# sIncerass/MVLPT

Measured on AMD Instinct MI355X. Metric: prompt-tuning images/sec (fwd+bwd), ViT-B/16 bs=256, 1/2/4/8 MI355X, higher is better.
Workload: dtype fp16; 1 GPU; BASELINE configs[1]: MVLPT coop head, ViT-B/16, 100 classes (caltech101 token table), n_ctx=16 n_vpt=0, text L=77, class token middle; text_positions_evaluated=77, step_pipelining=True, grad_precision=split_grad, layernorm_folding=both towers, residual_stream=packed fp16 + byte (image tower without prompts / backward), cu_partition=none (towers share every compute unit), per_gpu_batch=256, global_batch=256, parallelism=dp1, text_tower=replicated per GPU

## Files before the change

include/mvlpt_hip.h:

```cpp
#ifndef MVLPT_HIP_H
#define MVLPT_HIP_H
#include <stdint.h>
#ifdef __cplusplus
extern "C" {
#endif

typedef void* mvlpt_stream_t;

enum { MVLPT_DT_F32 = 0, MVLPT_DT_F16 = 1, MVLPT_DT_BF16 = 2 };
enum { MVLPT_LABEL_INT64 = 0, MVLPT_LABEL_PROB_F32 = 1 };
enum { MVLPT_ERR_ARG = -1, MVLPT_ERR_HIP = -2, MVLPT_ERR_STATE = -3, MVLPT_ERR_UNSUPPORTED = -4 };

typedef struct MvlptArch {
  int image_resolution, patch_size, vision_width, vision_layers, vision_heads;
  int context_length, text_width, text_layers, text_heads;
  int embed_dim;
  int compute_dtype;
} MvlptArch;

enum { MVLPT_PREC_FAST = 0, MVLPT_PREC_SPLIT_GRAD = 1, MVLPT_PREC_SPLIT_ALL = 2 };

int mvlpt_create(const MvlptArch* arch, void** handle);
int mvlpt_set_precision(void* handle, int mode);
int mvlpt_set_ln_fold(void* handle, int mode, int min_rows);
int mvlpt_set_resid_packed(void* handle, int on);
int mvlpt_set_vpt_dropout(void* handle, const float* masks, int n_layers, int batch, int n_vpt, int width);
int mvlpt_trim(void* handle);
int mvlpt_debug_checksums(void* handle, int enable, unsigned long long* host_out, int max_out);
int mvlpt_destroy(void* handle);
const char* mvlpt_last_error(void* handle);
const char* mvlpt_version(void);

int mvlpt_stream_create_cus(int cu_first, int cu_count, mvlpt_stream_t* stream);
int mvlpt_stream_destroy(mvlpt_stream_t stream);
int mvlpt_stream_cus(mvlpt_stream_t stream);

int mvlpt_load_frozen(void* handle, const char* name, const void* dev_ptr, int dtype, const int64_t* shape, int ndim,
                      mvlpt_stream_t stream);
int mvlpt_frozen_ready(void* handle);

int mvlpt_image_fwd(void* handle, const void* image, int image_dtype, const float* vpt, const float* vpt_deep, int n_vpt,
                    int n_deep, int B, float* feat_out, int save_for_bwd, mvlpt_stream_t stream);
int mvlpt_image_bwd(void* handle, const float* dfeat, float* dvpt, float* dvpt_deep, mvlpt_stream_t stream);

int mvlpt_text_fwd(void* handle, const float* prefix, const float* suffix, const float* ctx, int ctx_per_class, int n_ctx,
                   const int32_t* layout, const int32_t* eot, int C, int L, float* feat_out, int save_for_bwd,
                   mvlpt_stream_t stream);
int mvlpt_text_fwd_grouped(void* handle, const float* prefix, const float* suffix, const float* ctx, int n_ctx, const int32_t* layout,
                           const int32_t* eot, int G, int C, int L, float* feat_out, int save_for_bwd, mvlpt_stream_t stream);
int mvlpt_text_fwd_ranged(void* handle, const float* prefix, const float* suffix, const float* ctx, int n_ctx, const int32_t* layout,
                          const int32_t* eot, const int32_t* class_lo, const int32_t* class_hi, int G, int C, int L, float* feat_out,
                          int save_for_bwd, mvlpt_stream_t stream);
int mvlpt_text_bwd(void* handle, const float* dfeat, float* dctx, mvlpt_stream_t stream);
int mvlpt_text_workspace_bytes(void* handle, int C_total, int L, int save_for_bwd, int64_t* out);

enum { MVLPT_TEXT_MIN_L = 3 };
int mvlpt_text_encode_tokens(void* handle, const int32_t* ids, int ld, int S, int L, float* feat_out, mvlpt_stream_t stream);
int mvlpt_text_ensemble(const float* feats, int T, int C, int e, float* out, mvlpt_stream_t stream);

int mvlpt_logits_fwd(void* handle, const float* img_feat, const float* txt_feat, float logit_scale_exp, const int32_t* task_lo,
                     const int32_t* task_hi, int B, int C, float* logits, mvlpt_stream_t stream);
int mvlpt_logits_bwd(void* handle, const float* dlogits, float* dimg, float* dtxt, mvlpt_stream_t stream);
int mvlpt_logits_grouped_fwd(void* handle, const float* img, const float* txt, float logit_scale_exp, int G, int C, float* logits,
                             mvlpt_stream_t stream);
int mvlpt_logits_grouped_bwd(void* handle, const float* dlogits, float* dtxt, mvlpt_stream_t stream);
int mvlpt_logits_ranged_fwd(void* handle, const float* img, const float* txt, float logit_scale_exp, const int32_t* class_lo,
                            const int32_t* class_hi, int G, int C, float* logits, mvlpt_stream_t stream);
int mvlpt_logits_ranged_bwd(void* handle, const float* dlogits, float* dtxt, float* dimg, mvlpt_stream_t stream);

int mvlpt_cross_entropy(void* handle, const float* logits, const void* labels, int label_kind, int B, int C, float* loss,
                        float* dlogits, float* ncorrect, mvlpt_stream_t stream);

int mvlpt_op_gemm(int dtype, int epi, const void* A, const void* Bt, int M, int N, int K, const float* bias, const void* aux,
                  const float* resid, void* out, void* out2, mvlpt_stream_t stream);
int mvlpt_op_gemm_ex(int dtype, int epi, const void* A, const void* Bt, int M, int N, int K, const float* bias, const void* aux,
                     const float* resid, void* out, void* out2, int a_split, int lda, int ldo, int ldb, int w8_exp, int out_lo8,
                     mvlpt_stream_t stream);
enum { MVLPT_GEMM_BT_128x128_R2 = 1, MVLPT_GEMM_BT_128x128_R4 = 2, MVLPT_GEMM_BT_256x128_R3 = 3, MVLPT_GEMM_BT_256x256_R2 = 4,
       MVLPT_GEMM_PHASED = 5, MVLPT_GEMM_PC = 6, MVLPT_GEMM_PCP = 7 };
int mvlpt_op_gemm_route(int dtype, int epi, int a_split, int M, int N, int K, int fold_ntp, mvlpt_stream_t stream, int* tile_m,
                        int* tile_n, int* ring);
int mvlpt_op_gemm_split(int dtype, int epi, const void* A, const void* Bt, int M, int N, int K, const float* bias, const void* aux,
                        const float* resid, void* out, void* out2, mvlpt_stream_t stream);
int mvlpt_op_layernorm_fwd_split(int out_dtype, const float* x, const float* gamma, const float* beta, void* y, int rows, int d,
                                 mvlpt_stream_t stream);
int mvlpt_op_layernorm_bwd_split(int dtype, const void* dy, const float* x, const float* gamma, const float* resid, float* out32,
                                 void* out16, int rows, int d, mvlpt_stream_t stream);
int mvlpt_op_attention32_fwd(int dtype, const void* qkv, void* out, float* lse, int N, int L, int H, int causal, int q_rows,
                             mvlpt_stream_t stream);
int mvlpt_op_attention32_bwd(int dtype, const void* qkv, const void* out, const void* dout, const float* lse, float* delta,
                             void* dqkv, int N, int L, int H, int causal, mvlpt_stream_t stream);
int mvlpt_op_pack_weight_mixed(int dtype, const float* w32, int rows, int cols, int transposed, void* out, int* w8_exp,
                               mvlpt_stream_t stream);
int mvlpt_op_gemm_mixed(int dtype, int epi, const void* A, const void* Bt, int ldb, int w8_exp, int M, int N, int K, const float* bias,
                        const void* aux, const float* resid, void* out, void* out2, mvlpt_stream_t stream);
int mvlpt_op_cast_mixed(int dtype, const float* in, void* out, int64_t rows, int d, mvlpt_stream_t stream);
int mvlpt_op_fold_vectors(int dtype, const void* W16, int ld, const float* gamma, const float* beta, const float* b, float* colsum,
                          float* bias2, int N, int K, mvlpt_stream_t stream);
int mvlpt_op_gemm_ln_producer(int dtype, const void* A, int a_split, const void* Bt, int ldb, int w8_exp, int M, int N, int K,
                              const float* bias, const float* resid, const float* gamma, int x16_split, float* out32, void* x16,
                              float* part, int ntp, int* nt, mvlpt_stream_t stream);
int mvlpt_op_gemm_folded(int dtype, int epi, const void* A16, int a_split, const void* Bt, int ldb, int w8_exp, int M, int N, int K,
                         const float* colsum, const float* bias2, const float* part, int ntp, int nt, void* out, void* out2,
                         mvlpt_stream_t stream);
int mvlpt_op_fold_weight(const void* W16, int ld, const float* gamma, void* Wg16, int ldg, float* colsum, int N, int K,
                         mvlpt_stream_t stream);
int mvlpt_op_respk_pack(const float* x, void* hi, uint8_t* lo, float* part, int ntp, int rows, int d, mvlpt_stream_t stream);
int mvlpt_op_assemble_packed(const float* patch_emb, const float* cls, const float* pos, const float* ln_g, const float* ln_b, void* hi,
                             uint8_t* lo, float* part, int ntp, int batch, int grid2, int d, mvlpt_stream_t stream);
int mvlpt_op_respk_unpack(const void* hi, const uint8_t* lo, int row_mul, float* out, int rows, int d, mvlpt_stream_t stream);
int mvlpt_op_gemm_residp(const void* A, const void* Bt, int ldb, int M, int N, int K, const float* bias, const void* hi_in,
                         const uint8_t* lo_in, void* hi_out, uint8_t* lo_out, float* part, int ntp, int* nt, mvlpt_stream_t stream);
int mvlpt_op_layernorm_fwd_mixed(int out_dtype, const float* x, const float* gamma, const float* beta, void* y, int rows, int d,
                                 mvlpt_stream_t stream);
int mvlpt_op_layernorm_bwd_mixed(int dtype, const void* dy, const float* x, const float* gamma, const float* resid, float* out32,
                                 void* out16, int rows, int d, mvlpt_stream_t stream);
int mvlpt_op_attention32_fwd_mixed(int dtype, const void* qkv, void* out, float* lse, int N, int L, int H, int causal, int q_rows,
                                   mvlpt_stream_t stream);
int mvlpt_op_attention32_bwd_mixed(int dtype, const void* qkv, const void* out, const void* dout, const float* lse, float* delta,
                                   void* dqkv, int N, int L, int H, int causal, mvlpt_stream_t stream);
int mvlpt_op_layernorm_fwd(int out_dtype, const float* x, const float* gamma, const float* beta, void* y, int rows, int d,
                           mvlpt_stream_t stream);
int mvlpt_op_layernorm_bwd(int dtype, const void* dy, const float* x, const float* gamma, const float* resid, float* out32,
                           void* out16, int rows, int d, mvlpt_stream_t stream);
int mvlpt_op_attention_fwd(int dtype, const void* qkv, void* out, float* lse, int N, int L, int H, int causal,
// ... 77 lines not shown
```

mvlpt_amd/_lib.py:

```python
from __future__ import annotations

import ctypes as C
import os

import torch

_HERE = os.path.dirname(os.path.abspath(__file__))
LIB_PATH = os.environ.get("MVLPT_HIP_LIB") or os.path.join(_HERE, "libmvlpt_hip.so")

DT_F32, DT_F16, DT_BF16 = 0, 1, 2
LABEL_INT64, LABEL_PROB_F32 = 0, 1
EPI_STORE16, EPI_GELU, EPI_RESID32, EPI_GELUBWD, EPI_STORE32, EPI_GELU_SPLIT, EPI_GELUBWD_SPLIT, EPI_STORE_SPLIT = 0, 1, 2, 3, 4, 5, 6, 7
GEMM_BT_128x128_R2, GEMM_BT_128x128_R4, GEMM_BT_256x128_R3, GEMM_BT_256x256_R2, GEMM_PHASED, GEMM_PC, GEMM_PCP = 1, 2, 3, 4, 5, 6, 7
PREC_FAST, PREC_SPLIT_GRAD, PREC_SPLIT_ALL = 0, 1, 2
TEXT_MIN_L = 3


class MvlptArch(C.Structure):
    _fields_ = [(n, C.c_int) for n in (
        "image_resolution", "patch_size", "vision_width", "vision_layers", "vision_heads",
        "context_length", "text_width", "text_layers", "text_heads", "embed_dim", "compute_dtype")]


class MvlptKernelStat(C.Structure):
    _fields_ = [("name", C.c_char * 32), ("launches", C.c_int64), ("ms", C.c_double),
                ("flops", C.c_double), ("bytes", C.c_double), ("busy_ms", C.c_double), ("flops_executed", C.c_double)]


class MvlptImageDesc(C.Structure):
    _fields_ = [("offset", C.c_int64)] + [(n, C.c_int32) for n in (
        "height", "width", "crop_top", "crop_left", "crop_height", "crop_width", "resize_height", "resize_width",
        "out_top", "out_left", "flip", "reserved")]


OPTIM_SGD, OPTIM_ADAM, OPTIM_ADAMW = 0, 1, 2
OPTIM_MAX_SEGS = 1024


class MvlptOptimSeg(C.Structure):
    _fields_ = [("begin", C.c_int64), ("end", C.c_int64), ("active", C.c_int32), ("missed", C.c_int32)]


class MvlptOptimHyper(C.Structure):
    _fields_ = [("kind", C.c_int32), ("nesterov", C.c_int32), ("lr", C.c_double), ("weight_decay", C.c_double), ("momentum", C.c_double),
                ("dampening", C.c_double), ("beta1", C.c_double), ("beta2", C.c_double), ("eps", C.c_double), ("launch", C.c_int64)]


_vp, _i, _f = C.c_void_p, C.c_int, C.c_float

SIGNATURES = {
    "mvlpt_create": (_i, [C.POINTER(MvlptArch), C.POINTER(_vp)]),
    "mvlpt_destroy": (_i, [_vp]),
    "mvlpt_set_precision": (_i, [_vp, _i]),
    "mvlpt_trim": (_i, [_vp]),
    "mvlpt_debug_checksums": (_i, [_vp, _i, C.POINTER(C.c_uint64), _i]),
    "mvlpt_set_ln_fold": (_i, [_vp, _i, _i]),
    "mvlpt_set_resid_packed": (_i, [_vp, _i]),
    "mvlpt_set_vpt_dropout": (_i, [_vp, _vp, _i, _i, _i, _i]),
    "mvlpt_last_error": (C.c_char_p, [_vp]),
    "mvlpt_version": (C.c_char_p, []),
    "mvlpt_stream_create_cus": (_i, [_i, _i, C.POINTER(_vp)]),
    "mvlpt_stream_destroy": (_i, [_vp]),
    "mvlpt_stream_cus": (_i, [_vp]),
    "mvlpt_load_frozen": (_i, [_vp, C.c_char_p, _vp, _i, C.POINTER(C.c_int64), _i, _vp]),
    "mvlpt_frozen_ready": (_i, [_vp]),
    "mvlpt_image_fwd": (_i, [_vp, _vp, _i, _vp, _vp, _i, _i, _i, _vp, _i, _vp]),
    "mvlpt_image_bwd": (_i, [_vp, _vp, _vp, _vp, _vp]),
    "mvlpt_text_fwd": (_i, [_vp, _vp, _vp, _vp, _i, _i, _vp, _vp, _i, _i, _vp, _i, _vp]),
    "mvlpt_text_bwd": (_i, [_vp, _vp, _vp, _vp]),
    "mvlpt_text_fwd_grouped": (_i, [_vp, _vp, _vp, _vp, _i, _vp, _vp, _i, _i, _i, _vp, _i, _vp]),
    "mvlpt_text_fwd_ranged": (_i, [_vp, _vp, _vp, _vp, _i, _vp, _vp, _vp, _vp, _i, _i, _i, _vp, _i, _vp]),
    "mvlpt_text_workspace_bytes": (_i, [_vp, _i, _i, _i, C.POINTER(C.c_int64)]),
    "mvlpt_text_encode_tokens": (_i, [_vp, _vp, _i, _i, _i, _vp, _vp]),
    "mvlpt_text_ensemble": (_i, [_vp, _i, _i, _i, _vp, _vp]),
    "mvlpt_logits_fwd": (_i, [_vp, _vp, _vp, _f, _vp, _vp, _i, _i, _vp, _vp]),
    "mvlpt_logits_bwd": (_i, [_vp, _vp, _vp, _vp, _vp]),
    "mvlpt_logits_grouped_fwd": (_i, [_vp, _vp, _vp, _f, _i, _i, _vp, _vp]),
    "mvlpt_logits_grouped_bwd": (_i, [_vp, _vp, _vp, _vp]),
    "mvlpt_logits_ranged_fwd": (_i, [_vp, _vp, _vp, _f, _vp, _vp, _i, _i, _vp, _vp]),
    "mvlpt_logits_ranged_bwd": (_i, [_vp, _vp, _vp, _vp, _vp]),
    "mvlpt_cross_entropy": (_i, [_vp, _vp, _vp, _i, _i, _i, _vp, _vp, _vp, _vp]),
    "mvlpt_op_gemm": (_i, [_i, _i, _vp, _vp, _i, _i, _i, _vp, _vp, _vp, _vp, _vp, _vp]),
    "mvlpt_op_gemm_ex": (_i, [_i, _i, _vp, _vp, _i, _i, _i, _vp, _vp, _vp, _vp, _vp, _i, _i, _i, _i, _i, _i, _vp]),
    "mvlpt_op_gemm_route": (_i, [_i, _i, _i, _i, _i, _i, _i, _vp, C.POINTER(_i), C.POINTER(_i), C.POINTER(_i)]),
    "mvlpt_op_gemm_split": (_i, [_i, _i, _vp, _vp, _i, _i, _i, _vp, _vp, _vp, _vp, _vp, _vp]),
    "mvlpt_op_layernorm_fwd_split": (_i, [_i, _vp, _vp, _vp, _vp, _i, _i, _vp]),
    "mvlpt_op_layernorm_bwd_split": (_i, [_i, _vp, _vp, _vp, _vp, _vp, _vp, _i, _i, _vp]),
    "mvlpt_op_attention32_fwd": (_i, [_i, _vp, _vp, _vp, _i, _i, _i, _i, _i, _vp]),
    "mvlpt_op_attention32_bwd": (_i, [_i, _vp, _vp, _vp, _vp, _vp, _vp, _i, _i, _i, _i, _vp]),
    "mvlpt_op_pack_weight_mixed": (_i, [_i, _vp, _i, _i, _i, _vp, C.POINTER(C.c_int), _vp]),
    "mvlpt_op_gemm_mixed": (_i, [_i, _i, _vp, _vp, _i, _i, _i, _i, _i, _vp, _vp, _vp, _vp, _vp, _vp]),
    "mvlpt_op_cast_mixed": (_i, [_i, _vp, _vp, C.c_int64, _i, _vp]),
    "mvlpt_op_fold_vectors": (_i, [_i, _vp, _i, _vp, _vp, _vp, _vp, _vp, _i, _i, _vp]),
    "mvlpt_op_gemm_ln_producer": (_i, [_i, _vp, _i, _vp, _i, _i, _i, _i, _i, _vp, _vp, _vp, _i, _vp, _vp, _vp, _i, C.POINTER(C.c_int), _vp]),
    "mvlpt_op_gemm_folded": (_i, [_i, _i, _vp, _i, _vp, _i, _i, _i, _i, _i, _vp, _vp, _vp, _i, _i, _vp, _vp, _vp]),
    "mvlpt_op_fold_weight": (_i, [_vp, _i, _vp, _vp, _i, _vp, _i, _i, _vp]),
    "mvlpt_op_respk_pack": (_i, [_vp, _vp, _vp, _vp, _i, _i, _i, _vp]),
    "mvlpt_op_assemble_packed": (_i, [_vp, _vp, _vp, _vp, _vp, _vp, _vp, _vp, _i, _i, _i, _i, _vp]),
    "mvlpt_op_respk_unpack": (_i, [_vp, _vp, _i, _vp, _i, _i, _vp]),
    "mvlpt_op_gemm_residp": (_i, [_vp, _vp, _i, _i, _i, _i, _vp, _vp, _vp, _vp, _vp, _vp, _i, C.POINTER(C.c_int), _vp]),
    "mvlpt_op_layernorm_fwd_mixed": (_i, [_i, _vp, _vp, _vp, _vp, _i, _i, _vp]),
    "mvlpt_op_layernorm_bwd_mixed": (_i, [_i, _vp, _vp, _vp, _vp, _vp, _vp, _i, _i, _vp]),
    "mvlpt_op_attention32_fwd_mixed": (_i, [_i, _vp, _vp, _vp, _i, _i, _i, _i, _i, _vp]),
    "mvlpt_op_attention32_bwd_mixed": (_i, [_i, _vp, _vp, _vp, _vp, _vp, _vp, _i, _i, _i, _i, _vp]),
    "mvlpt_op_layernorm_fwd": (_i, [_i, _vp, _vp, _vp, _vp, _i, _i, _vp]),
    "mvlpt_op_layernorm_bwd": (_i, [_i, _vp, _vp, _vp, _vp, _vp, _vp, _i, _i, _vp]),
    "mvlpt_op_attention_fwd": (_i, [_i, _vp, _vp, _vp, _i, _i, _i, _i, _vp]),
    "mvlpt_op_attention_bwd": (_i, [_i, _vp, _vp, _vp, _vp, _vp, _vp, _i, _i, _i, _i, _vp]),
    "mvlpt_op_cast": (_i, [_i, _vp, _vp, C.c_int64, _vp]),
    "mvlpt_op_assemble_prompts_ranged": (_i, [_vp, _vp, _vp, _i, _vp, _vp, _vp, _vp, _vp, _i, _i, _i, _i, _vp]),
    "mvlpt_op_gather_ctx_grad_ranged": (_i, [_vp, _vp, _vp, _vp, _i, _i, _i, _i, _i, _vp, _vp]),
    "mvlpt_op_embed_tokens": (_i, [_vp, _vp, _vp, _i, _vp, _i, _i, _i, _vp]),
    "mvlpt_op_ensemble_features": (_i, [_vp, _vp, _i, _i, _i, _vp]),
    "mvlpt_op_normalize_rows": (_i, [_vp, _vp, _vp, _i, _i, _vp]),
    "mvlpt_op_sgemm_bt": (_i, [_vp, _vp, _vp, _i, _i, _i, _vp, _vp]),
    "mvlpt_op_grad_scale": (_i, [_vp, C.c_int64, _f, _vp, _vp]),
    "mvlpt_op_optim_step": (_i, [C.POINTER(MvlptOptimHyper), _vp, _vp, _vp, _vp, C.c_int64, _vp, _i, _vp, _vp, _vp]),
    "mvlpt_op_reduce_prompt_rows": (_i, [_i, _vp, _vp, _i, _i, _i, _i, _i, _vp, _vp, _i, _i, _vp, _vp]),
    "mvlpt_op_gather_ctx_grad": (_i, [_vp, _vp, _i, _i, _i, _i, _i, _vp, _vp, _vp]),
    "mvlpt_op_attention_bwd_cls": (_i, [_i, _vp, _vp, _vp, _vp, _vp, _i, _i, _i, _vp]),
    "mvlpt_op_copy_rows": (_i, [_vp, _vp, _vp, _i, _i, _i, _vp]),
    "mvlpt_op_overwrite_rows": (_i, [_vp, _i, _vp, _i, _i, _i, _vp, _vp]),
    "mvlpt_op_assemble_tokens": (_i, [_vp, _vp, _vp, _vp, _vp, _vp, _i, _vp, _vp, _i, _i, _i, _vp]),
    "mvlpt_op_assemble_prompts": (_i, [_vp, _vp, _vp, _i, _i, _vp, _vp, _vp, _vp, _vp, _vp, _i, _i, _i, _vp]),
    "mvlpt_preprocess": (_i, [_vp, _vp, C.c_int64, C.POINTER(MvlptImageDesc), _i, _i, _i, C.POINTER(_f), C.POINTER(_f), _vp, _i, _vp, _vp]),
    "mvlpt_profile_begin": (_i, [_vp, _i]),
    "mvlpt_profile_pause": (_i, [_vp, _i]),
    "mvlpt_profile_end": (_i, [_vp, C.POINTER(MvlptKernelStat), _i]),
}


def load_library(path: str = LIB_PATH) -> C.CDLL:
    if not os.path.isfile(path):
        raise ImportError(
            f"{path} not found: build the HIP extension first (`make` at the repo root, or "
            "`__graft_entry__.build()`); mvlpt_amd has no CPU fallback.")
    lib = C.CDLL(path)
    for name, (res, args) in SIGNATURES.items():
        fn = getattr(lib, name)
        fn.restype, fn.argtypes = res, args
    return lib


lib = load_library()


def last_error(handle=None) -> str:
    msg = lib.mvlpt_last_error(handle)
    return msg.decode() if msg else ""
# ... 6 lines not shown
```

mvlpt_amd/config.py:

```python
from __future__ import annotations

from typing import Any, Iterable


class CfgNode(dict):
    def __getattr__(self, k):
        try:
            return self[k]
        except KeyError as e:
            raise AttributeError(k) from e

    def __setattr__(self, k, v):
        self[k] = v

    def clone(self) -> "CfgNode":
        return CfgNode({k: (v.clone() if isinstance(v, CfgNode) else v) for k, v in self.items()})

    def merge_from_list(self, opts: Iterable[Any]) -> None:
        opts = list(opts)
        assert len(opts) % 2 == 0, "override list must be KEY VAL pairs"
        for key, val in zip(opts[0::2], opts[1::2]):
            node = self
            parts = key.split(".")
            for p in parts[:-1]:
                node = node[p]
            if parts[-1] not in node:
                raise KeyError(f"unknown config key {key}")
            old = node[parts[-1]]
            if isinstance(val, str) and not isinstance(old, str):
                if isinstance(old, bool):
                    val = val.lower() in ("1", "true", "yes")
                elif isinstance(old, list) and old and isinstance(old[0], str):
                    import json
                    val = [str(x) for x in json.loads(val)]
                elif isinstance(old, (list, tuple)):
                    val = type(old)(int(x) for x in val.strip("()[]").split(","))
                else:
                    val = type(old)(val)
            node[parts[-1]] = val


def get_cfg_default() -> CfgNode:
    CN = CfgNode
    cfg = CN()
    cfg.SEED = 1
    cfg.OUTPUT_DIR = "./output"
    cfg.MODEL = CN(BACKBONE=CN(NAME="ViT-B/16"), INIT_WEIGHTS="")
    cfg.INPUT = CN(SIZE=(224, 224))
    cfg.DATALOADER = CN(TRAIN_X=CN(BATCH_SIZE=32), TEST=CN(BATCH_SIZE=100), NUM_WORKERS=8)
    cfg.OPTIM = CN(NAME="sgd", LR=0.002, MAX_EPOCH=200, MOMENTUM=0.9, WEIGHT_DECAY=5e-4, SGD_DAMPNING=0.0,
                   SGD_NESTEROV=False, LR_SCHEDULER="cosine", WARMUP_EPOCH=1, WARMUP_TYPE="constant",
                   WARMUP_CONS_LR=1e-5, WARMUP_MIN_LR=1e-5,
                   FUSED=False)
    cfg.TRAIN = CN(PRINT_FREQ=5, CHECKPOINT_FREQ=0)
    cfg.TEST = CN(FINAL_MODEL="last_step", SPLIT="test", NO_TEST=False)
    cfg.TRAINER = CN(NAME="MVLPT", CUT_CONTEXTLEN=False, ACT_CKPT=1)
    cfg.TRAINER.MVLPT = CN(
        PREC="fp16", PROJECT_METHOD="transformer", PROJECT_DIM=128,
        VPT=CN(N_CTX=0, CSC=False, CTX_INIT="", DROPOUT=0.0, PROJECT=-1, DEEP=True),
        COOP=CN(N_CTX=0, CSC=False, CTX_INIT="", CLASS_TOKEN_POSITION="middle"),
        COCOOP=CN(N_CTX=0, CTX_INIT="", PREC="fp16"),
        COMPUTE_DTYPE="fp16",
        GRAD_PRECISION="split_grad",
        STEP_PIPELINING=True,
    )
    cfg.TRAINER.COCOOP = CN(N_CTX=16, CTX_INIT="", PREC="fp16")
    cfg.TRAINER.ZSCLIP = CN(TEMPLATES=["a photo of a {}."])
    cfg.DATASET = CN(NAME="synthetic", COOP=True, MULTITASK=False, MULTITASK_LABEL_PERTASK=False,
                     MULTITASK_EVALKEY="average", NUM_SHOTS=16)
    return cfg
```

mvlpt_amd/csrc/attention.hip:

```cpp
#include <hip/hip_ext.h>
#include "attn_common.h"

namespace mvlpt {

constexpr int ATT_MAX_NKT = 38;
int attn_max_len() { return ATT_MAX_NKT * 16; }

template <typename T, int NKT, bool CAUSAL>
__global__ __launch_bounds__(256) void attn_fwd_kernel(AttnArgs a) {
  extern __shared__ __attribute__((aligned(16))) char smem[];
  using v8 = typename Vec<T>::v8;
  using v4 = typename Vec<T>::v4;
  constexpr int LP = NKT * 16;
  constexpr int BLK = NKT < 16 ? NKT : 16;
  constexpr bool PRELOAD = NKT <= 16;
  char* sK = smem;
  char* sV = smem + LP * 128;
  const int L = a.L, H = a.H, d = H * 64;
  const int n = blockIdx.x / H, h = blockIdx.x % H;
  const size_t ld = (size_t)3 * d;
  const T* base = (const T*)a.qkv + (size_t)n * L * ld + h * 64;
  const int lane = threadIdx.x & 63, wave = __builtin_amdgcn_readfirstlane(threadIdx.x >> 6);
  const int fr = lane & 15, fg = lane >> 4;
  const int nqt = a.q_rows > 0 ? ((a.q_rows < L ? a.q_rows : L) + 15) >> 4 : (L + 15) >> 4;
// ... 547 lines not shown
  if (tid < 64) gbase[tid] = from_f32<T>(red[0][tid] + red[1][tid] + red[2][tid] + red[3][tid]);
}

hipError_t launch_attn_bwd_cls(int dtype, const void* qkv, const void* o_cls, const void* do_cls, const float* lse, void* dqkv,
                               int N, int L, int H, hipStream_t s) {
  if (N <= 0 || L <= 0 || H <= 0) return hipErrorInvalidValue;
  if (dtype == DT_F16)
    hipLaunchKernelGGL(attn_bwd_cls_kernel<f16>, dim3(N * H), dim3(256), 0, s, (const f16*)qkv, (const f16*)o_cls, (const f16*)do_cls, lse,
                       (f16*)dqkv, N, L, H);
  else if (dtype == DT_BF16)
    hipLaunchKernelGGL(attn_bwd_cls_kernel<bf16>, dim3(N * H), dim3(256), 0, s, (const bf16*)qkv, (const bf16*)o_cls, (const bf16*)do_cls,
                       lse, (bf16*)dqkv, N, L, H);
  else return hipErrorInvalidValue;
  return hipGetLastError();
}

static thread_local hipEvent_t t_ev_a = nullptr, t_ev_b = nullptr;
template <typename T, int NKT, bool CAUSAL>
static hipError_t fwd_t(const AttnArgs& a, hipStream_t s) {
  constexpr int LP = NKT * 16;
  constexpr int lds = 2 * LP * 128;
  static bool set = false;
  if (!set) { hipFuncSetAttribute((const void*)attn_fwd_kernel<T, NKT, CAUSAL>, hipFuncAttributeMaxDynamicSharedMemorySize, lds); set = true; }
  hipExtLaunchKernelGGL((attn_fwd_kernel<T, NKT, CAUSAL>), dim3(a.N * a.H), dim3(256), lds, s, t_ev_a, t_ev_b, 0, a);
  return hipGetLastError();
}
template <typename T, int NKT, bool CAUSAL>
static hipError_t bwd_t(const AttnBwdArgs& a, hipStream_t s) {
  constexpr int LP = NKT * 16;
  constexpr int lds_a = 2 * LP * 128;
  constexpr int lds_b = 2 * LP * 128 + 2 * LP * 4;
  static bool set = false;
  if (!set) {
    hipFuncSetAttribute((const void*)attn_bwd_dq_kernel<T, NKT, CAUSAL>, hipFuncAttributeMaxDynamicSharedMemorySize, lds_a);
    hipFuncSetAttribute((const void*)attn_bwd_dkv_kernel<T, NKT, CAUSAL>, hipFuncAttributeMaxDynamicSharedMemorySize, lds_b);
    set = true;
  }
  hipLaunchKernelGGL((attn_bwd_dq_kernel<T, NKT, CAUSAL>), dim3(a.N * a.H), dim3(256), lds_a, s, a);
  hipError_t e = hipGetLastError();
  if (e != hipSuccess) return e;
  hipLaunchKernelGGL((attn_bwd_dkv_kernel<T, NKT, CAUSAL>), dim3(a.N * a.H), dim3(256), lds_b, s, a);
  return hipGetLastError();
}

#define MVLPT_NKT_SWITCH(FN, ARGS)                                  \
  switch (nkt) {                                                    \
    case 2: return FN<T, 2, CAUSAL> ARGS;                           \
    case 4: return FN<T, 4, CAUSAL> ARGS;                           \
    case 6: return FN<T, 6, CAUSAL> ARGS;                           \
    case 8: return FN<T, 8, CAUSAL> ARGS;                           \
    case 10: return FN<T, 10, CAUSAL> ARGS;                         \
    case 12: return FN<T, 12, CAUSAL> ARGS;                         \
    case 14: return FN<T, 14, CAUSAL> ARGS;                         \
    case 16: return FN<T, 16, CAUSAL> ARGS;                         \
  }                                                                 \
  if constexpr (!CAUSAL) {    \
    if (nkt == 18) return FN<T, 18, CAUSAL> ARGS;                   \
    if (nkt == 38) return FN<T, 38, CAUSAL> ARGS;                   \
  }                                                                 \
  return hipErrorInvalidValue;

template <typename T, bool CAUSAL> static hipError_t fwd_n(int nkt, const AttnArgs& a, hipStream_t s) {
  if constexpr (!CAUSAL) { if (nkt == 13) return fwd_t<T, 13, CAUSAL>(a, s); }
  MVLPT_NKT_SWITCH(fwd_t, (a, s))
}
template <typename T, bool CAUSAL> static hipError_t bwd_n(int nkt, const AttnBwdArgs& a, hipStream_t s) { MVLPT_NKT_SWITCH(bwd_t, (a, s)) }

static int nkt_for(int L) {
  int t = (L + 15) / 16; t += t & 1;
  if (t > 18) return 38;
  return t < 2 ? 2 : t;
}

static bool use_stream(int L) { return L > 256; }

hipError_t launch_attn_fwd(int dtype, const AttnArgs& a_, hipStream_t s, hipEvent_t ea, hipEvent_t eb) {
  t_ev_a = ea; t_ev_b = eb;
  AttnArgs a = a_;
  a.flags = 3;
  if (a.L <= 0 || a.L > attn_max_len() || a.N <= 0) return hipErrorInvalidValue;
  if (use_stream(a.L)) return launch_attn_fwd_stream(dtype, a, s);
  if (!a.causal && a.q_rows <= 0 && (a.L + 15) / 16 == PNT && (dtype == DT_F16 || dtype == DT_BF16)) {
    const int total = a.N * a.H, cus = stream_cus(s);
    if (total >= 2 * cus) {
      static bool set = false;
      if (!set) {
        hipFuncSetAttribute((const void*)attn_fwdp_kernel<f16>, hipFuncAttributeMaxDynamicSharedMemorySize, PLDS);
        hipFuncSetAttribute((const void*)attn_fwdp_kernel<bf16>, hipFuncAttributeMaxDynamicSharedMemorySize, PLDS);
        set = true;
      }
      if (dtype == DT_F16) hipExtLaunchKernelGGL((attn_fwdp_kernel<f16>), dim3(cus), dim3(PNW * 64), PLDS, s, ea, eb, 0, a, total);
      else hipExtLaunchKernelGGL((attn_fwdp_kernel<bf16>), dim3(cus), dim3(PNW * 64), PLDS, s, ea, eb, 0, a, total);
      return hipGetLastError();
    }
  }
  const int nkt = !a.causal && (a.L + 15) / 16 == 13 ? 13 : nkt_for(a.L);
  if (dtype == DT_F16) return a.causal ? fwd_n<f16, true>(nkt, a, s) : fwd_n<f16, false>(nkt, a, s);
  if (dtype == DT_BF16) return a.causal ? fwd_n<bf16, true>(nkt, a, s) : fwd_n<bf16, false>(nkt, a, s);
  return hipErrorInvalidValue;
}
hipError_t launch_attn_bwd(int dtype, const AttnBwdArgs& a, hipStream_t s) {
  if (a.L <= 0 || a.L > attn_max_len() || a.N <= 0) return hipErrorInvalidValue;
  if (use_stream(a.L)) return launch_attn_bwd_stream(dtype, a, s);
  const int nkt = nkt_for(a.L);
  if (dtype == DT_F16) return a.causal ? bwd_n<f16, true>(nkt, a, s) : bwd_n<f16, false>(nkt, a, s);
  if (dtype == DT_BF16) return a.causal ? bwd_n<bf16, true>(nkt, a, s) : bwd_n<bf16, false>(nkt, a, s);
  return hipErrorInvalidValue;
}

}
```

mvlpt_amd/csrc/attention32.hip:

```cpp
#include "attn_common.h"

namespace mvlpt {

#ifdef MVLPT_ATTN_TRACE
constexpr int ATR_MAX = 256;
#define MVLPT_ATR(p) do { if (a.trace && blockIdx.x == 1024 && lane == 0 && atr_n < ATR_MAX) \
    a.trace[wave * ATR_MAX + atr_n++] = ((long long)(p) << 56) | ((long long)__builtin_amdgcn_s_memtime() & 0xffffffffffffffLL); } while (0)
#define MVLPT_ATRB(p) do { if (a.trace && blockIdx.x == 5 && blockIdx.y == (gridDim.y >> 1) && lane == 0 && atr_n < ATR_MAX) \
    a.trace[wave * ATR_MAX + atr_n++] = ((long long)(p) << 56) | ((long long)__builtin_amdgcn_s_memtime() & 0xffffffffffffffLL); } while (0)
#else
#define MVLPT_ATR(p) do { } while (0)
#define MVLPT_ATRB(p) do { } while (0)
#endif

namespace {
constexpr int CH = 64;
constexpr int XIMG = CH * 128;
constexpr float SCALE = 0.125f;

template <typename T>
__device__ __forceinline__ void store_pair4(T* p, size_t lo_off, f32x4 v) {
  typename Vec<T>::v4 hi, lo;
#pragma unroll
  for (int e = 0; e < 4; ++e) { T h, l; split16<T>(v[e], h, l); hi[e] = h; lo[e] = l; }
// ... 1060 lines not shown
        __builtin_amdgcn_sched_barrier(0);
        if (dt + 1 < 4) load_v(kb, dt + 1, vn);
        else if (kb + 1 < (RNT + 1) / 2) load_v(kb + 1, 0, vn);
        __builtin_amdgcn_sched_barrier(0);
        if (2 * kb < nt) {
#pragma unroll
          for (int o = 0; o < 2; ++o) {
            O[o][dt] = mfma16<T>(vf[0], ph[o], O[o][dt]);
            O[o][dt] = mfma16<T>(vf[0], pl[o], O[o][dt]);
            O[o][dt] = mfma16<T>(vf[1], ph[o], O[o][dt]);
          }
        }
        __builtin_amdgcn_sched_barrier(0);
        vf[0] = vn[0]; vf[1] = vn[1];
      }
    }
#pragma unroll
    for (int o = 0; o < 2; ++o) {
      if (o == 1 && !two) continue;
      const int q = (wave + o * RNW) * 16 + fr;
      const bool ok = q < qlim;
      const int qc = ok ? q : 0;
      const float inv = 1.f / sum[o];
      T* orow = (T*)a.out_split + ((size_t)n * L + qc) * (2 * (size_t)d) + h * 64;
      if (ok) {
#pragma unroll
        for (int dt = 0; dt < 4; ++dt) store_pair4_m<T>(orow + 16 * dt + 4 * fg, d, h * 64 + 16 * dt + 4 * fg, O[o][dt] * inv, a.out_lo8);
        if (a.lse && fg == 0) a.lse[((size_t)n * a.H + h) * L + q] = mx[o] * SCALE + logf(sum[o]);
      }
    }
    kbuf = kbuf + 2 >= 3 ? kbuf - 1 : kbuf + 2;
  }
}

static bool attn32_resident(int L, int causal) { return !causal && L <= RROWS; }

static int attn32_nw(int rows) {
  const int pad8 = (rows + 255) / 256 * 256, pad4 = (rows + 127) / 128 * 128;
  return pad8 * 8 <= pad4 * 9 ? 8 : 4;
}
template <typename K>
static void set_lds(K kernel, int bytes) { (void)hipFuncSetAttribute((const void*)kernel, hipFuncAttributeMaxDynamicSharedMemorySize, bytes); }

template <typename T, bool CAUSAL, int NW>
static hipError_t fwd_x(const Attn32Args& a, hipStream_t s) {
  const int lq = a.q_rows > 0 ? (a.q_rows < a.L ? a.q_rows : a.L) : a.L;
  const int nqc = (lq + NW * 32 - 1) / (NW * 32);
  constexpr int lds = 8 * XIMG;
  static bool set = false;
  if (!set) { set_lds(attn32x_fwd_kernel<T, CAUSAL, NW>, lds); set = true; }
  hipLaunchKernelGGL((attn32x_fwd_kernel<T, CAUSAL, NW>), dim3(stream_grid(a.N * a.H, nqc)), dim3(NW * 64), lds, s, a, nqc);
  return hipGetLastError();
}
template <typename T, bool CAUSAL, int NW>
static hipError_t bwd_x(const Attn32BwdArgs& a, hipStream_t s) {
  const int nc = (a.L + NW * 32 - 1) / (NW * 32), lpad = (a.L + CH - 1) / CH * CH;
  constexpr int lds = 8 * XIMG;
  const int lds_kv = lds + 8 * lpad;
  static int set = 0;
  if (set < lds_kv) {
    set_lds(attn32x_dq_kernel<T, CAUSAL, NW>, lds); set_lds(attn32x_dkv_kernel<T, CAUSAL, NW>, lds_kv);
    set_lds(attn32x_bwd_fused_kernel<T, CAUSAL, NW>, lds_kv); set = lds_kv;
  }
  const dim3 grid(stream_grid(a.N * a.H, nc)), block(NW * 64);
  if (nc == 1) {
    hipLaunchKernelGGL((attn32x_bwd_fused_kernel<T, CAUSAL, NW>), grid, block, lds_kv, s, a, lpad);
    return hipGetLastError();
  }
  hipLaunchKernelGGL((attn32x_dq_kernel<T, CAUSAL, NW>), grid, block, lds, s, a, nc);
  hipLaunchKernelGGL((attn32x_dkv_kernel<T, CAUSAL, NW>), grid, block, lds_kv, s, a, nc, lpad);
  return hipGetLastError();
}

template <typename T>
static hipError_t fwd_t(const Attn32Args& a, hipStream_t s) {
  if (a.L <= SROWS) {
    dim3 grid(a.H, a.N), block(SNT * 64);
    if (a.causal) hipLaunchKernelGGL((attn32t_fwd_kernel<T, true>), grid, block, 0, s, a);
    else hipLaunchKernelGGL((attn32t_fwd_kernel<T, false>), grid, block, 0, s, a);
    return hipGetLastError();
  }
  if (attn32_resident(a.L, a.causal)) {
    const int total = a.N * a.H, cus = stream_cus(s);
    if (a.q_rows <= 0 && total >= 2 * cus) {
      static bool setp = false;
      if (!setp) { set_lds(attn32p_fwd_kernel<T>, RLDS_P); setp = true; }
      hipLaunchKernelGGL((attn32p_fwd_kernel<T>), dim3(cus), dim3(RNW * 64), RLDS_P, s, a, total);
      return hipGetLastError();
    }
    static bool set = false;
    if (!set) { set_lds(attn32r_fwd_kernel<T>, RLDS); set = true; }
    hipLaunchKernelGGL((attn32r_fwd_kernel<T>), dim3(a.H, a.N), dim3(RNW * 64), RLDS, s, a);
    return hipGetLastError();
  }
  const int lq = a.q_rows > 0 ? (a.q_rows < a.L ? a.q_rows : a.L) : a.L;
  if (attn32_nw(lq) == 8) return a.causal ? fwd_x<T, true, 8>(a, s) : fwd_x<T, false, 8>(a, s);
  return a.causal ? fwd_x<T, true, 4>(a, s) : fwd_x<T, false, 4>(a, s);
}
template <typename T>
static hipError_t bwd_t(const Attn32BwdArgs& a, hipStream_t s) {
  if (a.L <= SROWS) {
    dim3 grid(a.H, a.N), block(SNT * 64);
    if (a.causal) hipLaunchKernelGGL((attn32t_bwd_kernel<T, true>), grid, block, 0, s, a);
    else hipLaunchKernelGGL((attn32t_bwd_kernel<T, false>), grid, block, 0, s, a);
    return hipGetLastError();
  }
  if (attn32_resident(a.L, a.causal)) {
    static bool set = false;
    if (!set) { set_lds(attn32r_bwd_kernel<T>, RLDS_BWD); set = true; }
    hipLaunchKernelGGL((attn32r_bwd_kernel<T>), dim3(a.H, a.N), dim3(RNW * 64), RLDS_BWD, s, a);
    return hipGetLastError();
  }
  if (a.L > 8192) return hipErrorInvalidValue;
  if (attn32_nw(a.L) == 8) return a.causal ? bwd_x<T, true, 8>(a, s) : bwd_x<T, false, 8>(a, s);
  return a.causal ? bwd_x<T, true, 4>(a, s) : bwd_x<T, false, 4>(a, s);
}

hipError_t launch_attn32_fwd(int dtype, const Attn32Args& a, hipStream_t s) {
  if (a.L <= 0 || a.N <= 0 || a.H <= 0 || !a.qkv_split || !a.out_split) return hipErrorInvalidValue;
  if (dtype == DT_F16) return fwd_t<f16>(a, s);
  if (dtype == DT_BF16) return fwd_t<bf16>(a, s);
  return hipErrorInvalidValue;
}
hipError_t launch_attn32_bwd(int dtype, const Attn32BwdArgs& a, hipStream_t s) {
  if (a.L <= 0 || a.N <= 0 || a.H <= 0 || !a.qkv_split || !a.out_split || !a.dout_split || !a.lse || !a.delta || !a.dqkv_split)
    return hipErrorInvalidValue;
  if (dtype == DT_F16) return bwd_t<f16>(a, s);
  if (dtype == DT_BF16) return bwd_t<bf16>(a, s);
  return hipErrorInvalidValue;
}

}
```

mvlpt_amd/csrc/engine.hip:

```cpp
#include <hip/hip_runtime.h>

#include <cmath>
#include <cstdio>
#include <algorithm>
#include <array>
#include <map>
#include <cstring>
#include <mutex>
#include <string>
#include <vector>

#include "../../include/mvlpt_hip.h"
#include "kernels.h"

using namespace mvlpt;


namespace {
struct StreamPart { hipStream_t s; int cus; };
std::mutex g_part_mu;
std::vector<StreamPart> g_parts;
int device_cus() {
  static int cus = 0;
  if (!cus) {
    int dev = 0;
    (void)hipGetDevice(&dev);
    if (hipDeviceGetAttribute(&cus, hipDeviceAttributeMultiprocessorCount, dev) != hipSuccess || cus <= 0) cus = 256;
  }
  return cus;
}
}
namespace mvlpt {
int stream_cus(hipStream_t s) {
  if (s) {
    std::lock_guard<std::mutex> lk(g_part_mu);
    for (const StreamPart& p : g_parts) if (p.s == s) return p.cus;
  }
  return device_cus();
}
}

namespace {

struct DevBuf {
  void* p = nullptr;
  size_t cap = 0;
  std::vector<void*> retired;
  ~DevBuf() {
    if (p) (void)hipFree(p);
    for (void* q : retired) (void)hipFree(q);
  }
  size_t trim() {
    size_t n = retired.size();
    for (void* q : retired) (void)hipFree(q);
    retired.clear();
    return n;
  }
  hipError_t reserve(size_t bytes) {
    if (bytes <= cap) return hipSuccess;
    size_t got = std::max(bytes, cap + cap / 2);
    void* q = nullptr;
    hipError_t e = hipMalloc(&q, got);
    if (e != hipSuccess && got > bytes) { got = bytes; e = hipMalloc(&q, got); }
    if (e != hipSuccess) return e;
    if (p) retired.push_back(p);
    p = q; cap = got;
    return hipSuccess;
  }
};
struct Bump {
  char* base = nullptr; size_t off = 0, cap = 0;
  template <typename T> T* take(size_t count) {
    size_t bytes = (count * sizeof(T) + 255) & ~(size_t)255;
    T* r = (T*)(base + off); off += bytes; return r;
  }
  void* take_bytes(size_t bytes) { return take<char>(bytes); }
};
static size_t align256(size_t b) { return (b + 255) & ~(size_t)255; }

struct WRef { const void* p; int ld; int e8; };
struct Linear {
  void* w = nullptr; void* wt = nullptr; float* b = nullptr; int out = 0, in = 0;
  int ldw = 0, ldwt = 0, e8 = 0;
  float *fold_s = nullptr, *fold_b = nullptr;
  void* wg = nullptr; float* fold_sg = nullptr;
  WRef fw() const { return WRef{w, ldw, e8}; }
  WRef fwg() const { return WRef{wg, in, 0}; }
  WRef bw() const { return WRef{wt, ldwt, e8}; }
};
struct LNp { float* g = nullptr; float* b = nullptr; };
struct Block { LNp ln1, ln2; Linear qkv, o, fc, pr; };
struct TowerW { int width = 0, layers = 0, heads = 0; std::vector<Block> blocks; };

struct TowerState {
  bool valid = false, saved = false, causal = false;
  bool exact = false;
  int wide_pitch = 0;
  int xs = 0;
  int N = 0, L = 0, d = 0, H = 0, layers = 0;
  std::vector<float*> x;
  std::vector<void*> qkv, attn, u;
  std::vector<float*> lse;
  void *h16 = nullptr, *a16 = nullptr;
  float* dx32 = nullptr; void *dx16 = nullptr, *du16 = nullptr, *dO16 = nullptr, *dqkv16 = nullptr; float* dh32 = nullptr;
  float* delta = nullptr; float* scale_dev = nullptr;
  std::vector<char> skip;
  bool fold = false;
  float* part[2] = {nullptr, nullptr};
  int nt[2] = {0, 0}, ntp[2] = {0, 0};
};
constexpr int FOLD_NTP = 8;

enum ProfClass { PC_GEMM = 0, PC_ATTN_FWD, PC_ATTN_BWD, PC_LN_FWD, PC_LN_BWD, PC_GLUE, PC_HEAD, PC_ATTN_FWD_IMG, PC_COUNT };
static const char* kProfNames[PC_COUNT] = {"gemm_bt", "attention_fwd", "attention_bwd", "layernorm_fwd", "layernorm_bwd",
                                           "glue", "head_logits_ce", "attention_fwd_image"};
struct ProfRec { int cls; hipEvent_t a, b; double flops, bytes, flops_exec; int M = 0, N = 0, K = 0, epi = -1, split = 0, fold = 0; };

enum class TextKind { Plain, Ranged, Ids };
enum class HeadKind { Plain, Grouped, Ranged };

struct Engine {
  MvlptArch arch{};
  int dt = DT_F16;
  int prec_mode = MVLPT_PREC_SPLIT_GRAD;
  int fold_mode = 2;
  int fold_min_rows = 1024;
  bool fold_ready = false;
  int resid_packed = 1;
  const float* vpt_mask = nullptr;
  int vpt_mask_layers = 0, vpt_mask_B = 0, vpt_mask_n = 0, vpt_mask_d = 0;
  const float* v_mask = nullptr;
  bool lo8 = true;
  std::string err;
  TowerW vis, txt;
  void* conv_w = nullptr; int Kp = 0; float* cls_emb = nullptr; float* vpos = nullptr; LNp ln_pre, ln_post;
  float *vproj = nullptr, *vproj_t = nullptr;
  float* tpos = nullptr; LNp ln_final; float *tproj = nullptr, *tproj_t = nullptr;
  float* tok_emb = nullptr; int vocab = 0;
  std::vector<void*> owned;
  DevBuf vis_ws, txt_ws, head_ws, ce_ws, tmp, pp_ws;
  TowerState vs, ts;
  int vB = 0, v_nvpt = 0, v_ndeep = 0; float* cls32 = nullptr; float* dcls32 = nullptr;
  float* xc32 = nullptr; void *ac16 = nullptr, *hc16 = nullptr, *gc16 = nullptr;
  bool v_cls_last = false; float *xcm32 = nullptr, *xco32 = nullptr, *dxc32 = nullptr, *dhc32 = nullptr;
  void *uc16 = nullptr, *duc16 = nullptr, *dxc16 = nullptr, *dOc16 = nullptr;
  int tC = 0, tL = 0, t_nctx = 0, t_per_class = 0; int32_t* eot_rows = nullptr; int32_t* ctx_pos = nullptr;
  TextKind t_kind = TextKind::Plain;
  int t_groups = 0; const int32_t *t_rlo = nullptr, *t_rstart = nullptr;
  std::vector<int32_t> t_range_host, h_range_host;
  std::vector<int32_t> t_ids_host;
  bool t_eot_last = false; float *txc32 = nullptr, *txm32 = nullptr, *txo32 = nullptr, *tdxc32 = nullptr, *tdhc32 = nullptr;
  void *tac16 = nullptr, *thc16 = nullptr, *tgc16 = nullptr, *tuc16 = nullptr, *tduc16 = nullptr, *tdxc16 = nullptr, *tdOc16 = nullptr;
  float* eot32 = nullptr; float* deot32 = nullptr;
  int hB = 0, hC = 0; float h_scale = 0.f; const int32_t *h_lo = nullptr, *h_hi = nullptr;
  HeadKind h_kind = HeadKind::Plain;
  int hS = 0; const int32_t *h_rlo = nullptr, *h_rstart = nullptr, *h_rgrp = nullptr;
  float *imn = nullptr, *txn = nullptr, *inorm = nullptr, *tnorm = nullptr;
  unsigned long long* dbg_ck = nullptr; int dbg_ck_n = 0; bool dbg_ck_on = false;
  bool prof_on = false, prof_all = false; std::vector<ProfRec> prof; std::vector<hipEvent_t> ev_pool; size_t ev_used = 0;
};

thread_local std::string g_create_err;

int fail(Engine* E, int code, const std::string& msg) { if (E) E->err = msg; else g_create_err = msg; return code; }
int hipfail(Engine* E, hipError_t e, const char* what) {
  return fail(E, MVLPT_ERR_HIP, std::string(what) + ": " + hipGetErrorString(e));
}
#define HIPCHK(E, call) do { hipError_t _e = (call); if (_e != hipSuccess) return hipfail((E), _e, #call); } while (0)

struct ProfScope {
  Engine* E; hipStream_t s; bool on = false; hipEvent_t b{};
  ProfScope(Engine* E_, hipStream_t s_, int cls, double flops, double bytes) : E(E_), s(s_) {
    if (!E || !E->prof_on || !E->prof_all) return;
    if (E->ev_used + 2 > E->ev_pool.size()) {
      if (E->ev_pool.size() >= 65536) return;
      for (int i = 0; i < 512; ++i) { hipEvent_t ev; if (hipEventCreate(&ev) != hipSuccess) return; E->ev_pool.push_back(ev); }
    }
    hipEvent_t a = E->ev_pool[E->ev_used++]; b = E->ev_pool[E->ev_used++];
    (void)hipEventRecord(a, s);
    E->prof.push_back(ProfRec{cls, a, b, flops, bytes, flops});
    on = true;
  }
  ~ProfScope() { if (on) (void)hipEventRecord(b, s); }
};

constexpr int DBG_CK_MAX = 256;
static void dbg_ck(Engine* E, const void* p, size_t bytes, hipStream_t s) {
  if (!E->dbg_ck_on || !E->dbg_ck || E->dbg_ck_n >= DBG_CK_MAX) return;
  (void)launch_checksum(p, bytes, E->dbg_ck + E->dbg_ck_n++, s);
}

static hipError_t attn_fwd_timed(Engine* E, const AttnArgs& a, double flops, double bytes, hipStream_t s) {
  hipEvent_t ea = nullptr, eb = nullptr;
  if (E && E->prof_on && !E->prof_all) {
    if (E->ev_used + 2 > E->ev_pool.size() && E->ev_pool.size() < 65536)
      for (int i = 0; i < 512; ++i) { hipEvent_t ev; if (hipEventCreate(&ev) != hipSuccess) break; E->ev_pool.push_back(ev); }
    if (E->ev_used + 2 <= E->ev_pool.size()) {
      ea = E->ev_pool[E->ev_used++]; eb = E->ev_pool[E->ev_used++];
      E->prof.push_back(ProfRec{PC_ATTN_FWD_IMG, ea, eb, flops, bytes, flops});
    }
  }
  return launch_attn_fwd(E->dt, a, s, ea, eb);
}

struct Fold {
  const float* ln_gamma = nullptr; void* ln_x16 = nullptr; int ln_split = 0; float* ln_part = nullptr; int ln_ntp = 0;
  const float* fold_part = nullptr; const float* fold_colsum = nullptr; int fold_ntp = 0, fold_nt = 0;
  const void* rp_hi_in = nullptr; const uint8_t* rp_lo_in = nullptr; uint8_t* rp_lo_out = nullptr;
};
hipError_t gemm(Engine* E, int epi, const void* A, WRef Bt, int M, int N, int K, const float* bias, const void* aux,
                const float* resid, void* out, void* out2, hipStream_t s, int dtype = -1, int a_split = 0, const Fold* f = nullptr,
                int lda = 0, int ldo = 0) {
  GemmArgs g{A, Bt.p, M, N, K, bias, aux, resid, out, out2};
  g.a_split = a_split; g.ldb = Bt.ld; g.w8_exp = Bt.e8; g.lda = lda; g.ldo = ldo;
  if (f) {
    g.ln_gamma = f->ln_gamma; g.ln_x16 = f->ln_x16; g.ln_split = f->ln_split; g.ln_part = f->ln_part; g.ln_ntp = f->ln_ntp;
    g.fold_part = f->fold_part; g.fold_colsum = f->fold_colsum; g.fold_ntp = f->fold_ntp; g.fold_nt = f->fold_nt;
    g.rp_hi_in = f->rp_hi_in; g.rp_lo_in = f->rp_lo_in; g.rp_lo_out = f->rp_lo_out;
  }
  g.out_lo8 = (a_split == 2 && (epi == EPI_GELU_SPLIT || epi == EPI_GELUBWD_SPLIT)) ? 1 : 0;
  const int dt = dtype >= 0 ? dtype : E->dt;
  const double ob = (epi == EPI_RESIDP_LN) ? 6.0 : (epi == EPI_RESID32) ? 8.0 : (epi == EPI_RESID32_LN) ? 8.0 + 2.0 * (a_split ? 1.5 : 1.0) : ((epi == EPI_STORE32 || epi == EPI_STORE_SPLIT) ? 4.0 : ((epi == EPI_GELUBWD || epi == EPI_GELU_SPLIT) ? 4.0 :
                    (epi == EPI_GELUBWD_SPLIT ? 6.0 : 2.0)));
  hipEvent_t ea = nullptr, eb = nullptr;
  if (E && E->prof_on) {
    if (E->ev_used + 2 > E->ev_pool.size() && E->ev_pool.size() < 65536)
// ... 335 lines not shown
      }
    }
  }
  HIPCHK(E, hipStreamSynchronize(s));
  E->fold_ready = true;
  return 0;
}

}

extern "C" {

#ifndef MVLPT_SRC_HASH
#define MVLPT_SRC_HASH "unknown"
#endif
#ifndef MVLPT_GIT_HASH
#define MVLPT_GIT_HASH "nogit"
#endif
const char* mvlpt_version(void) { return "mvlpt_hip 0.1 (gfx950) src:" MVLPT_SRC_HASH " git:" MVLPT_GIT_HASH; }

const char* mvlpt_last_error(void* h) { return h ? ((Engine*)h)->err.c_str() : g_create_err.c_str(); }

int mvlpt_create(const MvlptArch* a, void** handle) {
  if (!a || !handle) return fail(nullptr, MVLPT_ERR_ARG, "null argument");
  if (a->compute_dtype != MVLPT_DT_F16 && a->compute_dtype != MVLPT_DT_BF16)
    return fail(nullptr, MVLPT_ERR_ARG, "compute_dtype must be MVLPT_DT_F16 or MVLPT_DT_BF16");
  if (a->vision_width != a->vision_heads * 64 || a->text_width != a->text_heads * 64)
    return fail(nullptr, MVLPT_ERR_UNSUPPORTED, "head_dim must be 64 (CLIP ViT: heads = width // 64)");
  if (a->vision_width % 128 || a->text_width % 128 || a->embed_dim % 64)
    return fail(nullptr, MVLPT_ERR_UNSUPPORTED, "widths must be multiples of 128 and embed_dim of 64");
  if (a->patch_size <= 0 || a->image_resolution % a->patch_size)
    return fail(nullptr, MVLPT_ERR_ARG, "image_resolution must be a multiple of patch_size");
  if (a->vision_layers <= 0 || a->text_layers <= 0 || a->context_length <= 0)
    return fail(nullptr, MVLPT_ERR_ARG, "bad layer count / context length");
  int ndev = 0;
  if (hipGetDeviceCount(&ndev) != hipSuccess || ndev == 0)
    return fail(nullptr, MVLPT_ERR_HIP, "no HIP device visible: libmvlpt_hip needs an AMD GPU (there is no CPU fallback)");
  Engine* E = new Engine();
  E->arch = *a; E->dt = a->compute_dtype;
  if (const char* v = getenv("MVLPT_SPLIT_LO8")) E->lo8 = atoi(v) != 0;
  if (const char* v = getenv("MVLPT_LN_FOLD")) E->fold_mode = atoi(v);
  if (const char* v = getenv("MVLPT_RESID_PACKED")) E->resid_packed = atoi(v) ? 1 : 0;
  if (const char* v = getenv("MVLPT_LN_FOLD_MIN_ROWS")) E->fold_min_rows = atoi(v) > 0 ? atoi(v) : 1;
  E->vis.width = a->vision_width; E->vis.layers = a->vision_layers; E->vis.heads = a->vision_heads;
  E->vis.blocks.resize(a->vision_layers);
  E->txt.width = a->text_width; E->txt.layers = a->text_layers; E->txt.heads = a->text_heads;
  E->txt.blocks.resize(a->text_layers);
  const int K = 3 * a->patch_size * a->patch_size;
  E->Kp = (K + 63) / 64 * 64;
  *handle = E;
  return 0;
}

int mvlpt_set_precision(void* h, int mode) {
  Engine* E = (Engine*)h;
  if (!E) return MVLPT_ERR_ARG;
  if (mode != MVLPT_PREC_FAST && mode != MVLPT_PREC_SPLIT_GRAD && mode != MVLPT_PREC_SPLIT_ALL)
    return fail(E, MVLPT_ERR_ARG, "set_precision: unknown mode");
  E->prec_mode = mode;
  return 0;
}

int mvlpt_stream_create_cus(int cu_first, int cu_count, mvlpt_stream_t* stream) {
  if (!stream) return fail(nullptr, MVLPT_ERR_ARG, "stream_create_cus: null argument");
  const int total = device_cus();
  if (cu_first < 0 || cu_count <= 0 || cu_first + cu_count > total)
    return fail(nullptr, MVLPT_ERR_ARG, "stream_create_cus: CU range outside the device (" + std::to_string(total) + " compute units)");
  std::vector<uint32_t> mask((total + 31) / 32, 0u);
  for (int i = cu_first; i < cu_first + cu_count; ++i) mask[i >> 5] |= 1u << (i & 31);
  hipStream_t s = nullptr;
  hipError_t e = hipExtStreamCreateWithCUMask(&s, (uint32_t)mask.size(), mask.data());
  if (e != hipSuccess) return hipfail(nullptr, e, "hipExtStreamCreateWithCUMask");
  { std::lock_guard<std::mutex> lk(g_part_mu); g_parts.push_back(StreamPart{s, cu_count}); }
  *stream = (mvlpt_stream_t)s;
  return 0;
}

int mvlpt_stream_destroy(mvlpt_stream_t stream) {
  hipStream_t s = (hipStream_t)stream;
  if (!s) return 0;
  {
    std::lock_guard<std::mutex> lk(g_part_mu);
    for (size_t i = 0; i < g_parts.size(); ++i) if (g_parts[i].s == s) { g_parts.erase(g_parts.begin() + i); break; }
  }
  hipError_t e = hipStreamDestroy(s);
  if (e != hipSuccess) return hipfail(nullptr, e, "hipStreamDestroy");
  return 0;
}

int mvlpt_stream_cus(mvlpt_stream_t stream) { return stream_cus((hipStream_t)stream); }

int mvlpt_set_resid_packed(void* h, int on) {
  Engine* E = (Engine*)h;
  if (!E) return MVLPT_ERR_ARG;
  if ((on != 0) != (E->resid_packed != 0)) E->fold_ready = false;
  E->resid_packed = on ? 1 : 0;
  return 0;
}
int mvlpt_set_ln_fold(void* h, int mode, int min_rows) {
  Engine* E = (Engine*)h;
  if (!E) return MVLPT_ERR_ARG;
  if (mode < 0 || mode > 2 || min_rows < 1) return fail(E, MVLPT_ERR_ARG, "set_ln_fold: mode in {0, 1, 2}, min_rows >= 1");
  E->fold_mode = mode; E->fold_min_rows = min_rows;
  return 0;
}

int mvlpt_set_vpt_dropout(void* h, const float* masks, int n_layers, int batch, int n_vpt, int width) {
  Engine* E = (Engine*)h;
  if (!E) return MVLPT_ERR_ARG;
  if (masks && (n_layers <= 0 || batch <= 0 || n_vpt <= 0 || width != E->arch.vision_width))
    return fail(E, MVLPT_ERR_ARG, "set_vpt_dropout: masks are [n_layers, batch, n_vpt, vision_width], every extent positive");
  E->vpt_mask = masks;
  E->vpt_mask_layers = masks ? n_layers : 0;
  E->vpt_mask_B = masks ? batch : 0; E->vpt_mask_n = masks ? n_vpt : 0; E->vpt_mask_d = masks ? width : 0;
  return 0;
}

int mvlpt_debug_checksums(void* h, int enable, unsigned long long* host_out, int max_out) {
  Engine* E = (Engine*)h;
  if (!E) return MVLPT_ERR_ARG;
  int n = 0;
  if (host_out && max_out > 0 && E->dbg_ck) {
    HIPCHK(E, hipDeviceSynchronize());
    n = E->dbg_ck_n < max_out ? E->dbg_ck_n : max_out;
    HIPCHK(E, hipMemcpy(host_out, E->dbg_ck, (size_t)n * sizeof(unsigned long long), hipMemcpyDeviceToHost));
  }
  if (enable && !E->dbg_ck) {
    void* p = nullptr;
    HIPCHK(E, hipMalloc(&p, DBG_CK_MAX * sizeof(unsigned long long)));
    E->owned.push_back(p);
    E->dbg_ck = (unsigned long long*)p;
  }
  E->dbg_ck_on = enable != 0;
  return n;
}

int mvlpt_trim(void* h) {
  Engine* E = (Engine*)h;
  if (!E) return MVLPT_ERR_ARG;
  HIPCHK(E, hipDeviceSynchronize());
  for (DevBuf* b : {&E->vis_ws, &E->txt_ws, &E->head_ws, &E->ce_ws, &E->tmp, &E->pp_ws}) (void)b->trim();
  return 0;
}

int mvlpt_destroy(void* h) {
  if (!h) return 0;
  Engine* E = (Engine*)h;
  (void)hipDeviceSynchronize();
  for (void* p : E->owned) (void)hipFree(p);
  for (hipEvent_t ev : E->ev_pool) (void)hipEventDestroy(ev);
  delete E;
  return 0;
}

int mvlpt_load_frozen(void* h, const char* name, const void* dev_ptr, int dtype, const int64_t* shape, int ndim,
                      mvlpt_stream_t stream) {
  Engine* E = (Engine*)h;
  if (!E || !name || !dev_ptr || !shape || ndim < 0 || ndim > 4) return fail(E, MVLPT_ERR_ARG, "null/invalid argument");
  hipStream_t s = (hipStream_t)stream;
  size_t n = 1;
  for (int i = 0; i < ndim; ++i) n *= (size_t)shape[i];
  std::string nm(name);
  if (nm == "logit_scale") return 0;
  const bool is_tok = nm == "token_embedding.weight";
  if (!is_tok) E->fold_ready = false;
  const float* p32 = (const float*)dev_ptr;
  if (dtype != MVLPT_DT_F32) {
    HIPCHK(E, E->tmp.reserve(n * 4));
    HIPCHK(E, launch_cast_any_to_f32(dtype, dev_ptr, (float*)E->tmp.p, n, s));
    p32 = (const float*)E->tmp.p;
  }
  const MvlptArch& A = E->arch;
  const int dv = A.vision_width, dtw = A.text_width, e = A.embed_dim;
  const int G2 = (A.image_resolution / A.patch_size) * (A.image_resolution / A.patch_size);
  auto is1 = [&](int r) { return ndim == 1 && shape[0] == r; };
  auto is2 = [&](int r, int c) { return ndim == 2 && shape[0] == r && shape[1] == c; };
  int rc = 0;
  const char* vb = "visual.transformer.resblocks.";
  const char* tb = "transformer.resblocks.";
  if (nm.rfind(vb, 0) == 0 || nm.rfind(tb, 0) == 0) {
    const bool isv = nm.rfind(vb, 0) == 0;
    int layer; const char* tail;
    if (!parse_block_name(name + strlen(isv ? vb : tb), &layer, &tail)) return fail(E, MVLPT_ERR_ARG, "malformed block name: " + nm);
    rc = load_block_tensor(E, isv ? E->vis : E->txt, layer, tail, p32, shape, ndim, s);
  } else if (nm == "visual.conv1.weight") {
    if (!(ndim == 4 && shape[0] == dv && shape[1] == 3 && shape[2] == A.patch_size && shape[3] == A.patch_size))
      return fail(E, MVLPT_ERR_ARG, "shape mismatch: " + nm);
    void* w = nullptr;
    HIPCHK(E, hipMalloc(&w, (size_t)dv * E->Kp * 2)); E->owned.push_back(w);
    HIPCHK(E, launch_pack_weight(E->dt, p32, w, dv, 3 * A.patch_size * A.patch_size, E->Kp, s));
    E->conv_w = w;
  } else if (nm == "visual.class_embedding") { if (!is1(dv)) return fail(E, MVLPT_ERR_ARG, "shape mismatch: " + nm); rc = upload_f32(E, p32, n, &E->cls_emb, s);
  } else if (nm == "visual.positional_embedding") { if (!is2(G2 + 1, dv)) return fail(E, MVLPT_ERR_ARG, "shape mismatch: " + nm); rc = upload_f32(E, p32, n, &E->vpos, s);
  } else if (nm == "visual.ln_pre.weight") { if (!is1(dv)) return fail(E, MVLPT_ERR_ARG, "shape mismatch: " + nm); rc = upload_f32(E, p32, n, &E->ln_pre.g, s);
  } else if (nm == "visual.ln_pre.bias") { if (!is1(dv)) return fail(E, MVLPT_ERR_ARG, "shape mismatch: " + nm); rc = upload_f32(E, p32, n, &E->ln_pre.b, s);
  } else if (nm == "visual.ln_post.weight") { if (!is1(dv)) return fail(E, MVLPT_ERR_ARG, "shape mismatch: " + nm); rc = upload_f32(E, p32, n, &E->ln_post.g, s);
  } else if (nm == "visual.ln_post.bias") { if (!is1(dv)) return fail(E, MVLPT_ERR_ARG, "shape mismatch: " + nm); rc = upload_f32(E, p32, n, &E->ln_post.b, s);
  } else if (nm == "visual.proj") {
    if (!is2(dv, e)) return fail(E, MVLPT_ERR_ARG, "shape mismatch: " + nm);
    void *w = nullptr, *wt = nullptr;
    HIPCHK(E, hipMalloc(&w, n * 4)); E->owned.push_back(w);
    HIPCHK(E, hipMalloc(&wt, n * 4)); E->owned.push_back(wt);
    HIPCHK(E, launch_pack_weight(DT_F32, p32, w, dv, e, e, s));
    HIPCHK(E, launch_pack_weight_t(DT_F32, p32, wt, dv, e, s));
    E->vproj = (float*)w; E->vproj_t = (float*)wt;
  } else if (nm == "positional_embedding") { if (!is2(A.context_length, dtw)) return fail(E, MVLPT_ERR_ARG, "shape mismatch: " + nm); rc = upload_f32(E, p32, n, &E->tpos, s);
  } else if (nm == "ln_final.weight") { if (!is1(dtw)) return fail(E, MVLPT_ERR_ARG, "shape mismatch: " + nm); rc = upload_f32(E, p32, n, &E->ln_final.g, s);
  } else if (nm == "ln_final.bias") { if (!is1(dtw)) return fail(E, MVLPT_ERR_ARG, "shape mismatch: " + nm); rc = upload_f32(E, p32, n, &E->ln_final.b, s);
  } else if (is_tok) {
    if (!(ndim == 2 && shape[0] > 0 && shape[0] <= INT32_MAX && shape[1] == dtw)) return fail(E, MVLPT_ERR_ARG, "shape mismatch: " + nm);
    E->vocab = 0;
    rc = upload_f32(E, p32, n, &E->tok_emb, s);
    if (!rc) E->vocab = (int)shape[0];
  } else if (nm == "text_projection") {
    if (!is2(dtw, e)) return fail(E, MVLPT_ERR_ARG, "shape mismatch: " + nm);
    void *w = nullptr, *wt = nullptr;
    HIPCHK(E, hipMalloc(&w, n * 4)); E->owned.push_back(w);
    HIPCHK(E, hipMalloc(&wt, n * 4)); E->owned.push_back(wt);
    HIPCHK(E, launch_pack_weight(DT_F32, p32, w, dtw, e, e, s));
    HIPCHK(E, launch_pack_weight_t(DT_F32, p32, wt, dtw, e, s));
    E->tproj = (float*)w; E->tproj_t = (float*)wt;
  } else {
    return fail(E, MVLPT_ERR_ARG, "unknown frozen tensor name: " + nm);
  }
  if (rc) return rc;
  if (dtype != MVLPT_DT_F32) HIPCHK(E, hipStreamSynchronize(s));
  return 0;
}

int mvlpt_frozen_ready(void* h) {
  Engine* E = (Engine*)h;
  if (!E) return MVLPT_ERR_ARG;
  const char* m = first_missing(E);
  if (m) return fail(E, MVLPT_ERR_STATE, std::string("frozen tensor not loaded: ") + m);
  return 0;
}

int mvlpt_image_fwd(void* h, const void* image, int image_dtype, const float* vpt, const float* vpt_deep, int n_vpt, int n_deep,
                    int B, float* feat_out, int save_for_bwd, mvlpt_stream_t stream) {
  Engine* E = (Engine*)h;
  if (!E || !image || !feat_out || B <= 0) return fail(E, MVLPT_ERR_ARG, "image_fwd: null/invalid argument");
  if (int rc = mvlpt_frozen_ready(h)) return rc;
  if ((n_vpt > 0) != (vpt != nullptr)) return fail(E, MVLPT_ERR_ARG, "image_fwd: vpt pointer and n_vpt disagree");
  if ((n_deep > 0) != (vpt_deep != nullptr) || (n_deep > 0 && n_vpt <= 0)) return fail(E, MVLPT_ERR_ARG, "image_fwd: deep prompts need vpt");
  hipStream_t s = (hipStream_t)stream;
  const MvlptArch& A = E->arch;
  const int G = A.image_resolution / A.patch_size, G2 = G * G, dv = A.vision_width, e = A.embed_dim;
  const int Lv = 1 + n_vpt + G2;
  if (Lv > attn_max_len()) return fail(E, MVLPT_ERR_UNSUPPORTED, "image_fwd: sequence length > 256 not supported yet");
  const bool save = save_for_bwd != 0;
  const bool exact = E->prec_mode == MVLPT_PREC_SPLIT_ALL || (E->prec_mode == MVLPT_PREC_SPLIT_GRAD && save);
  const size_t X = exact ? 2 : 1;
  const size_t npatch = (size_t)B * G2;
  size_t need = tower_bytes(E->vis, B, Lv, save, exact) + align256(npatch * E->Kp * 2) + align256(npatch * dv * 4) +
                7 * align256((size_t)B * dv * 4) + 4 * align256((size_t)B * dv * 2 * X) + 3 * align256((size_t)B * dv * 8 * X) + 4096;
  E->vs.valid = false;
  HIPCHK(E, E->vis_ws.reserve(need));
  Bump bp; bp.base = (char*)E->vis_ws.p; bp.cap = E->vis_ws.cap;
  void* patches = bp.take_bytes(npatch * E->Kp * 2);
  float* pe = bp.take<float>(npatch * dv);
  E->cls32 = bp.take<float>((size_t)B * dv);
  E->dcls32 = bp.take<float>((size_t)B * dv);
  E->xc32 = bp.take<float>((size_t)B * dv);
  E->ac16 = bp.take_bytes((size_t)B * dv * 2 * X); E->hc16 = bp.take_bytes((size_t)B * dv * 2 * X);
  E->gc16 = bp.take_bytes((size_t)B * dv * 4 * 2 * X);
  E->xcm32 = bp.take<float>((size_t)B * dv); E->xco32 = bp.take<float>((size_t)B * dv);
  E->dxc32 = bp.take<float>((size_t)B * dv); E->dhc32 = bp.take<float>((size_t)B * dv);
  E->dxc16 = bp.take_bytes((size_t)B * dv * 2 * X); E->dOc16 = bp.take_bytes((size_t)B * dv * 2 * X);
  E->uc16 = bp.take_bytes((size_t)B * dv * 4 * 2); E->duc16 = bp.take_bytes((size_t)B * dv * 4 * 2 * X);
  E->v_cls_last = false;
  carve_tower(bp, E->vis, E->vs, B, Lv, save, false, exact, split_kind(E));
  TowerState& st = E->vs;
  E->vB = B; E->v_nvpt = n_vpt; E->v_ndeep = n_deep;
  st.fold = E->fold_mode >= 1 && (size_t)B * Lv >= (size_t)E->fold_min_rows && dv >= 256;
  if (st.fold) if (int rc = prepare_fold(E, s)) return rc;

  const float* const masks = E->vpt_mask;
  const int mask_layers = E->vpt_mask_layers, mask_B = E->vpt_mask_B, mask_n = E->vpt_mask_n;
  E->vpt_mask = nullptr; E->vpt_mask_layers = 0; E->v_mask = nullptr;
  if (masks && (n_vpt <= 0 || mask_layers < 1 + n_deep || mask_B != B || mask_n != n_vpt))
    return fail(E, MVLPT_ERR_ARG, "image_fwd: the prompt dropout masks do not match this forward (layers >= 1 + n_deep, batch, n_vpt)");
  E->v_mask = masks;
  auto vmask = [&](int l) -> const float* { return masks ? masks + (size_t)l * B * n_vpt * dv : nullptr; };
  { ProfScope ps(E, s, PC_GLUE, 0, (double)npatch * E->Kp * 6.0);
    HIPCHK(E, launch_patchify(E->dt, image, image_dtype, patches, B, A.image_resolution, A.patch_size, E->Kp, s)); }
  if (E->dbg_ck_on) { E->dbg_ck_n = 0; if (E->dbg_ck) (void)hipMemsetAsync(E->dbg_ck, 0, DBG_CK_MAX * sizeof(unsigned long long), s); }
  dbg_ck(E, patches, (size_t)npatch * E->Kp * 2, s);
  HIPCHK(E, gemm(E, EPI_STORE32, patches, WRef{E->conv_w, 0, 0}, (int)npatch, dv, E->Kp, nullptr, nullptr, nullptr, pe, nullptr, s));
  dbg_ck(E, pe, (size_t)npatch * dv * 4, s);
  const int nt_d = dv / 128, ntp_d = (nt_d + 1) & ~1;
  const bool packed = E->resid_packed && E->dt == DT_F16 && !save && !exact && st.fold && n_vpt == 0 && dv % 128 == 0 &&
                      ntp_d <= FOLD_NTP && E->vis.blocks[0].qkv.wg != nullptr;
  void* const xhi = st.x[0];
  uint8_t* const xlo = (uint8_t*)st.x[0] + (size_t)B * Lv * dv * 2;
  if (packed) {
    ProfScope ps(E, s, PC_GLUE, 0, (double)B * Lv * dv * 7.0);
    HIPCHK(E, launch_assemble_tokens_packed(pe, E->cls_emb, E->vpos, E->ln_pre.g, E->ln_pre.b, xhi, xlo, st.part[0], ntp_d, B, G2, dv, s));
    st.nt[0] = nt_d; st.ntp[0] = ntp_d;
    dbg_ck(E, xhi, (size_t)B * Lv * dv * 3, s); dbg_ck(E, st.part[0], (size_t)B * Lv * ntp_d * 8, s);
  } else {
    ProfScope ps(E, s, PC_GLUE, 0, (double)B * Lv * dv * 8.0);
    HIPCHK(E, launch_assemble_tokens(pe, E->cls_emb, E->vpos, E->ln_pre.g, E->ln_pre.b, vpt, n_vpt, st.x[0], B, G2, dv, s, vmask(0)));
  }
  bool cls_only_last = false;
  bool ln1_ready = packed;
  auto next_foldable = [&](int l) -> const LNp* {
    const int n = l + 1;
    if (!st.fold || n >= E->vis.layers) return nullptr;
    if (n_deep > 0) return nullptr;
    return &E->vis.blocks[n].ln1;
  };
  for (int l = 0; l < E->vis.layers; ++l) {
    if (l > 0 && n_deep > 0) {
      if (l <= n_deep) {
        ProfScope ps(E, s, PC_GLUE, 0, (double)B * n_vpt * dv * 4.0);
        HIPCHK(E, launch_overwrite_rows(vpt_deep + (size_t)(l - 1) * n_vpt * dv, n_vpt, st.x[2 * l], B, Lv, dv, s, vmask(l)));
      } else {
        st.skip[l] = 1;
        if (st.saved) {
          HIPCHK(E, hipMemcpyAsync(st.x[2 * l + 2], st.x[2 * l], (size_t)B * Lv * dv * 4, hipMemcpyDeviceToDevice, s));
        }
        continue;
      }
    }
    if (l == E->vis.layers - 1) { cls_only_last = true; break; }
    if (packed) { if (int rc = block_fwd_packed(E, E->vis, st, l, s)) return rc; continue; }
    bool produced = false;
    if (int rc = block_fwd(E, E->vis, st, l, s, ln1_ready, next_foldable(l), &produced)) return rc;
    ln1_ready = produced;
  }
  if (cls_only_last) {
    const int l = E->vis.layers - 1;
    const Block& Bk = E->vis.blocks[l];
    const int T = B * Lv;
    float* xin = st.x[2 * l];
    float* xmid = save ? E->xcm32 : E->xc32;
    float* xout = save ? E->xco32 : E->xc32;
    E->v_cls_last = save;
    const int xs = st.xs;
    Fold fq;
    if (ln1_ready) fq = fold_consumer(st, 0, Bk.qkv);
    else HIPCHK(E, ln_fwd(E, E->dt, xin, nullptr, 1, Bk.ln1, st.h16, T, dv, s, xs));
    if (packed) fq.fold_colsum = Bk.qkv.fold_sg;
    HIPCHK(E, gemm(E, xs ? EPI_STORE_SPLIT : EPI_STORE16, packed ? xhi : st.h16, packed ? Bk.qkv.fwg() : Bk.qkv.fw(), T, 3 * dv, dv,
                   ln1_ready ? Bk.qkv.fold_b : Bk.qkv.b, nullptr, nullptr, st.qkv[l], nullptr, s, -1, xs, ln1_ready ? &fq : nullptr));
    dbg_ck(E, st.qkv[l], (size_t)T * 3 * dv * 2 * X, s);
    if (xs) {
      if (save) HIPCHK(E, launch_zero(st.attn[l], (size_t)T * dv * 4, s));
      if (int rc = attn32_fwd(E, st, l, 1, s)) return rc;
    } else {
      AttnArgs a{st.qkv[l], st.attn[l], save ? st.lse[l] : nullptr, st.N, st.L, st.H, 0, 1};
      ProfScope ps(E, s, PC_ATTN_FWD, 4.0 * st.L * 64.0 * st.N * st.H, (double)T * dv * 2.0 * 2.0);
      HIPCHK(E, launch_attn_fwd(E->dt, a, s));
    }
    { ProfScope ps(E, s, PC_GLUE, 0, (double)B * dv * 12.0);
      HIPCHK(E, launch_copy_rows_strided(st.attn[l], E->ac16, B, (size_t)Lv * dv * 2 * X, (size_t)dv * 2 * X, (int)(dv * 2 * X), s));
      if (packed) HIPCHK(E, launch_respk_unpack_rows(xhi, xlo, Lv, E->xc32, B, dv, s));
      else HIPCHK(E, launch_copy_rows_strided(xin, E->xc32, B, (size_t)Lv * dv * 4, (size_t)dv * 4, dv * 4, s)); }
    dbg_ck(E, E->ac16, (size_t)B * dv * 2 * X, s); dbg_ck(E, E->xc32, (size_t)B * dv * 4, s);
    HIPCHK(E, gemm(E, EPI_RESID32, E->ac16, Bk.o.fw(), B, dv, dv, Bk.o.b, nullptr, E->xc32, xmid, nullptr, s, -1, xs));
    HIPCHK(E, ln_fwd(E, E->dt, xmid, nullptr, 1, Bk.ln2, E->hc16, B, dv, s, xs));
    HIPCHK(E, gemm(E, xs ? EPI_GELU_SPLIT : EPI_GELU, E->hc16, Bk.fc.fw(), B, 4 * dv, dv, Bk.fc.b, nullptr, nullptr, E->gc16, save ? E->uc16 : nullptr, s, -1, xs));
    HIPCHK(E, gemm(E, EPI_RESID32, E->gc16, Bk.pr.fw(), B, dv, 4 * dv, Bk.pr.b, nullptr, xmid, xout, nullptr, s, -1, xs));
    HIPCHK(E, ln_fwd(E, DT_F32, xout, nullptr, 1, E->ln_post, E->cls32, B, dv, s));
  } else
  HIPCHK(E, ln_fwd(E, DT_F32, st.x[2 * E->vis.layers], nullptr, Lv, E->ln_post, E->cls32, B, dv, s));
  { ProfScope ps(E, s, PC_HEAD, 2.0 * B * e * dv, 4.0 * ((double)B * dv + (double)e * dv + (double)B * e));
    HIPCHK(E, launch_sgemm_bt(E->cls32, E->vproj_t, feat_out, B, e, dv, nullptr, s)); }
  return 0;
}

int mvlpt_image_bwd(void* h, const float* dfeat, float* dvpt, float* dvpt_deep, mvlpt_stream_t stream) {
  Engine* E = (Engine*)h;
  if (!E || !dfeat) return fail(E, MVLPT_ERR_ARG, "image_bwd: null argument");
  TowerState& st = E->vs;
  if (!st.valid || !st.saved) return fail(E, MVLPT_ERR_STATE, "image_bwd: call image_fwd(save_for_bwd=1) first");
  if ((E->v_nvpt > 0 && !dvpt) || (E->v_ndeep > 0 && !dvpt_deep)) return fail(E, MVLPT_ERR_ARG, "image_bwd: missing gradient output");
  hipStream_t s = (hipStream_t)stream;
  const MvlptArch& A = E->arch;
  const int B = E->vB, dv = A.vision_width, e = A.embed_dim, Lv = st.L, n = E->v_nvpt;
  const size_t T = (size_t)B * Lv;
  { ProfScope ps(E, s, PC_GLUE, 0, (double)T * dv * 10.0);
    HIPCHK(E, launch_grad_scale(dfeat, (size_t)B * e, 64.0f, st.scale_dev, s));
    HIPCHK(E, launch_sgemm_bt(dfeat, E->vproj, E->dcls32, B, dv, e, st.scale_dev, s)); }
  { ProfScope ps(E, s, PC_GLUE, 0, (double)T * dv * 4.0);
    HIPCHK(E, launch_zero(st.dx32, T * dv * 4, s)); }
  int l_top = st.layers - 1;
  const int xs = st.xs;
  if (E->v_cls_last) {
    const int l = st.layers - 1;
    const Block& Bk = E->vis.blocks[l];
    const int Ti = (int)T;
    HIPCHK(E, ln_bwd(E, E->dcls32, DT_F32, E->xco32, nullptr, 1, E->ln_post, nullptr, E->dxc32, E->dxc16, B, dv, s, -1, xs));
    HIPCHK(E, gemm(E, xs ? EPI_GELUBWD_SPLIT : EPI_GELUBWD, E->dxc16, Bk.pr.bw(), B, 4 * dv, dv, nullptr, E->uc16, nullptr, E->duc16, nullptr, s, -1, xs));
    HIPCHK(E, gemm(E, EPI_STORE32, E->duc16, Bk.fc.bw(), B, dv, 4 * dv, nullptr, nullptr, nullptr, E->dhc32, nullptr, s, -1, xs));
    HIPCHK(E, ln_bwd(E, E->dhc32, DT_F32, E->xcm32, nullptr, 1, Bk.ln2, E->dxc32, E->dxc32, E->dxc16, B, dv, s, -1, xs));
    HIPCHK(E, gemm(E, xs ? EPI_STORE_SPLIT : EPI_STORE16, E->dxc16, Bk.o.bw(), B, dv, dv, nullptr, nullptr, nullptr, E->dOc16, nullptr, s, -1, xs));
    if (xs) {
      { ProfScope ps(E, s, PC_GLUE, 0, (double)T * dv * 4.0);
        HIPCHK(E, launch_zero(st.dO16, T * dv * 4, s));
        HIPCHK(E, launch_copy_rows_strided(E->dOc16, st.dO16, B, (size_t)dv * 4, (size_t)Lv * dv * 4, dv * 4, s)); }
      if (int rc = attn32_bwd(E, st, l, s)) return rc;
    } else {
      ProfScope ps(E, s, PC_ATTN_BWD, 10.0 * st.L * 64.0 * st.N * st.H, (double)T * dv * 2.0 * 5.0);
      HIPCHK(E, launch_attn_bwd_cls(E->dt, st.qkv[l], E->ac16, E->dOc16, st.lse[l], st.dqkv16, st.N, st.L, st.H, s)); }
    { ProfScope ps(E, s, PC_GLUE, 0, (double)B * dv * 8.0);
      HIPCHK(E, launch_copy_rows_strided(E->dxc32, st.dx32, B, (size_t)dv * 4, (size_t)Lv * dv * 4, dv * 4, s)); }
    HIPCHK(E, gemm(E, EPI_STORE32, st.dqkv16, Bk.qkv.bw(), Ti, dv, 3 * dv, nullptr, nullptr, nullptr, st.dh32, nullptr, s, -1, xs));
    HIPCHK(E, ln_bwd(E, st.dh32, DT_F32, st.x[2 * l], nullptr, 1, Bk.ln1, st.dx32, st.dx32, st.dx16, Ti, dv, s, -1, xs));
    if (l > 0 && E->v_ndeep > 0 && l <= E->v_ndeep) {
      ProfScope ps(E, s, PC_GLUE, 0, (double)B * n * dv * 10.0);
      HIPCHK(E, launch_reduce_prompt_rows(E->dt, st.dx32, st.dx16, B, Lv, dv, 1, n, dvpt_deep + (size_t)(l - 1) * n * dv,
                                          st.scale_dev, 1, s, xs, E->v_mask ? E->v_mask + (size_t)l * B * n * dv : nullptr));
    }
    l_top = l - 1;
  } else {
    HIPCHK(E, ln_bwd(E, E->dcls32, DT_F32, st.x[2 * st.layers], nullptr, Lv, E->ln_post, nullptr, st.dx32, nullptr, B, dv, s));
    { ProfScope ps(E, s, PC_GLUE, 0, (double)T * dv * 6.0);
      if (xs) HIPCHK(E, launch_cast_f32_split(E->dt, st.dx32, st.dx16, T, dv, nullptr, s, xs == 2));
      else HIPCHK(E, launch_cast_f32_to16(E->dt, st.dx32, st.dx16, T * dv, nullptr, s)); }
  }
  for (int l = l_top; l >= 0; --l) {
    if (st.skip[l]) continue;
    if (int rc = block_bwd(E, E->vis, st, l, s)) return rc;
    if (l > 0 && E->v_ndeep > 0 && l <= E->v_ndeep) {
      ProfScope ps(E, s, PC_GLUE, 0, (double)B * n * dv * 10.0);
      HIPCHK(E, launch_reduce_prompt_rows(E->dt, st.dx32, st.dx16, B, Lv, dv, 1, n, dvpt_deep + (size_t)(l - 1) * n * dv,
                                          st.scale_dev, 1, s, xs, E->v_mask ? E->v_mask + (size_t)l * B * n * dv : nullptr));
    }
  }
  if (n > 0) {
    ProfScope ps(E, s, PC_GLUE, 0, (double)B * n * dv * 4.0);
    HIPCHK(E, launch_reduce_prompt_rows(E->dt, st.dx32, st.dx16, B, Lv, dv, 1, n, dvpt, st.scale_dev, 0, s, 0, E->v_mask));
  }
  return 0;
}

static int64_t build_range_table(const int32_t* class_lo, const int32_t* class_hi, int G, int C, std::vector<int32_t>& t) {
  int64_t S = 0;
  for (int g = 0; g < G; ++g) {
    if (class_lo[g] < 0 || class_lo[g] > class_hi[g] || class_hi[g] > C) return -1;
    S += class_hi[g] - class_lo[g];
  }
  if (S > INT32_MAX) return -1;
  t.resize((size_t)2 * G + 1 + 2 * (size_t)S);
  int32_t *lo = t.data(), *start = lo + G, *cls = start + G + 1, *grp = cls + S;
  int32_t s = 0;
  for (int g = 0; g < G; ++g) {
    lo[g] = class_lo[g]; start[g] = s;
    for (int c = class_lo[g]; c < class_hi[g]; ++c, ++s) { cls[s] = c; grp[s] = g; }
  }
  start[G] = s;
  return S;
}

static size_t text_ws_bytes(Engine* E, int C, int L, bool save, bool exact, size_t ctx_rows) {
  const int dtw = E->arch.text_width;
  const size_t X = exact ? 2 : 1;
// ... 818 lines not shown
```

mvlpt_amd/csrc/kernels.h:

```cpp
#pragma once
#include "common.h"

struct MvlptOptimHyper;
struct MvlptOptimSeg;

namespace mvlpt {

int stream_cus(hipStream_t s);

enum GemmEpi {
  EPI_STORE16 = 0,
  EPI_GELU = 1,
  EPI_RESID32 = 2,
  EPI_GELUBWD = 3,
  EPI_STORE32 = 4,
  EPI_GELU_SPLIT = 5,
  EPI_GELUBWD_SPLIT = 6,
  EPI_STORE_SPLIT = 7,
  EPI_RESID32_LN = 8,
  EPI_STORE16_FOLD = 9, EPI_GELU_FOLD = 10, EPI_STORE_SPLIT_FOLD = 11, EPI_GELU_SPLIT_FOLD = 12,
  EPI_RESIDP_LN = 13,
};
constexpr int epi_base(int epi) {
  return epi == EPI_STORE16_FOLD ? EPI_STORE16 : epi == EPI_GELU_FOLD ? EPI_GELU : epi == EPI_STORE_SPLIT_FOLD ? EPI_STORE_SPLIT
         : epi == EPI_GELU_SPLIT_FOLD ? EPI_GELU_SPLIT : epi;
}
constexpr bool epi_folds(int epi) { return epi >= EPI_STORE16_FOLD && epi <= EPI_GELU_SPLIT_FOLD; }
constexpr bool epi_ln_producer(int epi) { return epi == EPI_RESID32_LN || epi == EPI_RESIDP_LN; }
struct GemmArgs {
  const void* A;
  const void* Bt;
  int M, N, K;
  const float* bias;
  const void* aux;
  const float* resid;
  void* out;
  void* out2;
  int a_split = 0;
  int ldb = 0;
  int w8_exp = 0;
  int out_lo8 = 0;
  int lda = 0, ldo = 0;
  int xcd_order = 0;
  const float* ln_gamma = nullptr;
  void* ln_x16 = nullptr;
  int ln_split = 0;
  float* ln_part = nullptr;
  int ln_ntp = 0;
  const float* fold_part = nullptr;
  const float* fold_colsum = nullptr;
  int fold_ntp = 0, fold_nt = 0;
  const void* rp_hi_in = nullptr;
  const uint8_t* rp_lo_in = nullptr;
  uint8_t* rp_lo_out = nullptr;
#ifdef MVLPT_GEMM_TRACE
  long long* trace = nullptr;
#endif
};
int gemm_tile_n(int dtype, int epi, const GemmArgs& g, hipStream_t s);
enum GemmFamily {
  GEMM_FAM_BT_128x128_R2 = 1,
  GEMM_FAM_BT_128x128_R4 = 2,
  GEMM_FAM_BT_256x128_R3 = 3,
  GEMM_FAM_BT_256x256_R2 = 4,
  GEMM_FAM_PHASED = 5,
  GEMM_FAM_PC = 6,
  GEMM_FAM_PCP = 7,
};
struct GemmRoute { int family = 0, tile_m = 0, tile_n = 0, ring = 0; };
hipError_t gemm_route(int dtype, int epi, const GemmArgs& g, bool folded, hipStream_t s, GemmRoute* r);
hipError_t launch_gemm(int dtype, int epi, const GemmArgs& g, hipStream_t s, hipEvent_t ev_start = nullptr,
                       hipEvent_t ev_stop = nullptr);

hipError_t launch_sgemm_bt(const float* A, const float* Bt, float* C, int M, int N, int K, const float* alpha_dev, hipStream_t s);

struct LnFwdArgs {
  const float* x; const int32_t* row_idx; int row_mul;
  const float* gamma; const float* beta;
  void* y;
  int rows, d;
  int split = 0;
};
hipError_t launch_ln_fwd(int out_dtype, const LnFwdArgs& a, hipStream_t s);

struct LnBwdArgs {
  const void* dy;
  int dy_dtype;
  const float* x; const int32_t* row_idx; int row_mul;
  const float* gamma;
  const float* resid;
  float* out32;
// ... 120 lines not shown
```

mvlpt_amd/engine.py:

```python
from __future__ import annotations

import ctypes as C
from typing import Dict, List, Optional, Tuple

import torch

from . import _lib
from ._lib import DT_BF16, DT_F16, DT_F32, lib
from .weights import ClipArch, arch_from_state_dict

_TORCH2DT = {torch.float32: DT_F32, torch.float16: DT_F16, torch.bfloat16: DT_BF16}
_DT2TORCH = {DT_F16: torch.float16, DT_BF16: torch.bfloat16, DT_F32: torch.float32}


def _ptr(t: Optional[torch.Tensor]):
    return None if t is None else C.c_void_p(t.data_ptr())


def _stream() -> C.c_void_p:
    return C.c_void_p(torch.cuda.current_stream().cuda_stream)


def _on_device(fn):
    import functools

    @functools.wraps(fn)
    def wrapped(self, *a, **k):
        if torch.cuda.current_device() == self.device.index:
            return fn(self, *a, **k)
        with torch.cuda.device(self.device):
            return fn(self, *a, **k)
    return wrapped


_PARTITION_STREAMS: Dict[Tuple[int, int, int], "torch.cuda.ExternalStream"] = {}


def partition_stream(device: torch.device, cu_first: int, cu_count: int) -> "torch.cuda.Stream":
    key = (device.index, cu_first, cu_count)
    st = _PARTITION_STREAMS.get(key)
    if st is None:
        h = C.c_void_p()
        with torch.cuda.device(device):
            _lib.check(lib.mvlpt_stream_create_cus(cu_first, cu_count, C.byref(h)), None, "stream_create_cus")
        st = _PARTITION_STREAMS[key] = torch.cuda.ExternalStream(h.value, device=device)
    return st


def device_cus(device: torch.device) -> int:
    with torch.cuda.device(device):
        return int(lib.mvlpt_stream_cus(None))


def _host_ranges(class_lo, class_hi, G: int, n_cls: int):
    if any(isinstance(t, torch.Tensor) and t.is_cuda for t in (class_lo, class_hi)):
        raise ValueError("class ranges are host arrays (a device tensor would have to be read back)")
    lo = [int(v) for v in (class_lo.tolist() if hasattr(class_lo, "tolist") else class_lo)]
    hi = [int(v) for v in (class_hi.tolist() if hasattr(class_hi, "tolist") else class_hi)]
    if len(lo) != G or len(hi) != G:
        raise ValueError(f"class ranges must have one entry per group ({G}), got {len(lo)} / {len(hi)}")
    if any(not (0 <= a <= b <= n_cls) for a, b in zip(lo, hi)):
        raise ValueError(f"class ranges must satisfy 0 <= lo <= hi <= {n_cls}")
    S = sum(b - a for a, b in zip(lo, hi))
    if S == 0:
        raise ValueError("every class range is empty")
    return (C.c_int32 * G)(*lo), (C.c_int32 * G)(*hi), S


def _req(t: torch.Tensor, dtype, name: str) -> torch.Tensor:
    if not t.is_cuda:
        raise RuntimeError(f"{name} must be a CUDA/HIP tensor: mvlpt_amd has no CPU path")
    if t.dtype != dtype:
        t = t.to(dtype)
    return t.contiguous()


class Engine:

    def __init__(self, arch: ClipArch, compute_dtype: str = "fp16", device: Optional[torch.device] = None):
        if not torch.cuda.is_available():
            raise RuntimeError("mvlpt_amd.Engine needs a HIP device (no CPU fallback)")
        self.device = torch.device(device if device is not None else f"cuda:{torch.cuda.current_device()}")
        if self.device.index is None:
            self.device = torch.device(f"cuda:{torch.cuda.current_device()}")
        self.arch = arch
        self.dt = {"fp16": DT_F16, "bf16": DT_BF16}[compute_dtype]
        self.torch_dtype = _DT2TORCH[self.dt]
        a = _lib.MvlptArch(arch.image_resolution, arch.vision_patch_size, arch.vision_width, arch.vision_layers,
                           arch.vision_heads, arch.context_length, arch.transformer_width, arch.transformer_layers,
                           arch.transformer_heads, arch.embed_dim, self.dt)
        h = C.c_void_p()
        with torch.cuda.device(self.device):
            _lib.check(lib.mvlpt_create(C.byref(a), C.byref(h)), None, "mvlpt_create")
        self.h = h
        self.precision = _lib.PREC_SPLIT_GRAD
        self._keep: List[torch.Tensor] = []
        self._img_state = None
        self._txt_state = None
        self._head_state = None

    def close(self):
        if getattr(self, "h", None):
            lib.mvlpt_destroy(self.h)
            self.h = None

    def __del__(self):
        try:
            self.close()
        except Exception:
            pass

    def set_precision(self, mode) -> None:
        code = {"fast": _lib.PREC_FAST, "split_grad": _lib.PREC_SPLIT_GRAD, "split_all": _lib.PREC_SPLIT_ALL}.get(mode, mode)
        _lib.check(lib.mvlpt_set_precision(self.h, int(code)), self.h, "set_precision")
        self.precision = int(code)

    def set_vpt_dropout(self, masks: Optional[torch.Tensor]) -> None:
        if masks is not None:
            masks = _req(masks, torch.float32, "vpt dropout masks")
            if masks.dim() != 4 or masks.shape[-1] != self.arch.vision_width:
                raise ValueError("vpt dropout masks must be [n_layers, B, n_vpt, vision_width]")
        self._vpt_masks = masks
        sh = (0, 0, 0, 0) if masks is None else tuple(int(v) for v in masks.shape)
        _lib.check(lib.mvlpt_set_vpt_dropout(self.h, _ptr(masks), *sh), self.h, "set_vpt_dropout")

    def debug_checksums(self, enable: bool = True):
        buf = (C.c_uint64 * 256)()
        n = lib.mvlpt_debug_checksums(self.h, int(bool(enable)), buf, 256)
        if n < 0:
            raise RuntimeError(_lib.last_error(self.h))
        return [int(buf[i]) for i in range(n)]

    def set_ln_fold(self, mode: int, min_rows: int = 1024) -> None:
        _lib.check(lib.mvlpt_set_ln_fold(self.h, int(mode), int(min_rows)), self.h, "set_ln_fold")

    def set_resid_packed(self, on: bool) -> None:
        _lib.check(lib.mvlpt_set_resid_packed(self.h, int(bool(on))), self.h, "set_resid_packed")

    @_on_device
    def trim(self) -> None:
        _lib.check(lib.mvlpt_trim(self.h), self.h, "trim")

    @classmethod
    def from_state_dict(cls, sd: Dict[str, torch.Tensor], compute_dtype: str = "fp16", device=None,
                        arch: Optional[ClipArch] = None) -> "Engine":
        eng = cls(arch or arch_from_state_dict(sd), compute_dtype, device)
        eng.load_frozen(sd)
        return eng

    def load_frozen(self, sd: Dict[str, torch.Tensor]) -> None:
        with torch.cuda.device(self.device):
            for name, t in sd.items():
                if name in ("logit_scale", "token_embedding.weight", "input_resolution", "context_length", "vocab_size"):
                    continue
                if t.dtype not in _TORCH2DT:
                    t = t.float()
                tg = t.to(self.device).contiguous()
                shape = (C.c_int64 * max(tg.dim(), 1))(*tg.shape)
                _lib.check(lib.mvlpt_load_frozen(self.h, name.encode(), _ptr(tg), _TORCH2DT[tg.dtype], shape, tg.dim(),
                                                 _stream()), self.h, f"load_frozen({name})")
                torch.cuda.current_stream().synchronize()
            _lib.check(lib.mvlpt_frozen_ready(self.h), self.h, "frozen_ready")

    @_on_device
    def image_fwd(self, image: torch.Tensor, vpt: Optional[torch.Tensor] = None, vpt_deep: Optional[torch.Tensor] = None,
                  save_for_bwd: bool = False) -> torch.Tensor:
        if image.dtype not in _TORCH2DT:
            image = image.float()
        image = image.contiguous()
        if not image.is_cuda:
            raise RuntimeError("image must be on the GPU")
        B = image.shape[0]
        n_vpt = n_deep = 0
        if vpt is not None:
            vpt = _req(vpt, torch.float32, "vpt").reshape(-1, self.arch.vision_width)
            n_vpt = vpt.shape[0]
        m = getattr(self, "_vpt_masks", None)
        if m is not None and (m.shape[1] != B or m.shape[2] != n_vpt):
            raise ValueError(f"vpt dropout masks are {tuple(m.shape)} but the batch has {B} images and {n_vpt} prompt tokens")
        if vpt_deep is not None:
            vpt_deep = _req(vpt_deep, torch.float32, "vpt_deep")
            n_deep = vpt_deep.shape[0]
        feat = torch.empty(B, self.arch.embed_dim, device=image.device, dtype=torch.float32)
        _lib.check(lib.mvlpt_image_fwd(self.h, _ptr(image), _TORCH2DT[image.dtype], _ptr(vpt), _ptr(vpt_deep), n_vpt, n_deep, B,
                                       _ptr(feat), int(save_for_bwd), _stream()), self.h, "image_fwd")
        self._img_state = (n_vpt, n_deep, B) if save_for_bwd else None
        self._vpt_masks_saved, self._vpt_masks = (m if save_for_bwd else None), None
        return feat

    @_on_device
    def image_bwd(self, dfeat: torch.Tensor) -> Tuple[Optional[torch.Tensor], Optional[torch.Tensor]]:
        if self._img_state is None:
            raise RuntimeError("image_bwd without image_fwd(save_for_bwd=True)")
        n_vpt, n_deep, B = self._img_state
        dfeat = _req(dfeat, torch.float32, "dfeat")
        dv = self.arch.vision_width
        dvpt = torch.empty(n_vpt, dv, device=dfeat.device, dtype=torch.float32) if n_vpt else None
        ddeep = torch.empty(n_deep, n_vpt, dv, device=dfeat.device, dtype=torch.float32) if n_deep else None
        _lib.check(lib.mvlpt_image_bwd(self.h, _ptr(dfeat), _ptr(dvpt), _ptr(ddeep), _stream()), self.h, "image_bwd")
        return dvpt, ddeep

    @_on_device
    def text_fwd(self, prefix: torch.Tensor, suffix: torch.Tensor, ctx: Optional[torch.Tensor], layout: torch.Tensor,
                 eot: torch.Tensor, save_for_bwd: bool = False) -> torch.Tensor:
        prefix = _req(prefix, torch.float32, "token_prefix")
        suffix = _req(suffix, torch.float32, "token_suffix")
        layout = _req(layout, torch.int32, "layout")
        eot = _req(eot, torch.int32, "eot")
        Cn, L = layout.shape
        per_class, n_ctx = 0, 0
        if ctx is not None:
            ctx = _req(ctx, torch.float32, "ctx")
            per_class = int(ctx.dim() == 3)
            n_ctx = ctx.shape[-2]
        feat = torch.empty(Cn, self.arch.embed_dim, device=prefix.device, dtype=torch.float32)
        _lib.check(lib.mvlpt_text_fwd(self.h, _ptr(prefix), _ptr(suffix), _ptr(ctx), per_class, n_ctx, _ptr(layout), _ptr(eot),
                                      Cn, L, _ptr(feat), int(save_for_bwd), _stream()), self.h, "text_fwd")
        self._txt_state = (tuple(ctx.shape) if ctx is not None else None, layout, eot) if save_for_bwd else None
        return feat

    @_on_device
    def text_fwd_grouped(self, prefix: torch.Tensor, suffix: torch.Tensor, ctx: torch.Tensor, layout: torch.Tensor,
                         eot: torch.Tensor, save_for_bwd: bool = False) -> torch.Tensor:
        prefix = _req(prefix, torch.float32, "token_prefix")
        suffix = _req(suffix, torch.float32, "token_suffix")
        layout = _req(layout, torch.int32, "layout")
        eot = _req(eot, torch.int32, "eot")
        ctx = _req(ctx, torch.float32, "ctx")
        if ctx.dim() != 3:
            raise ValueError("grouped ctx must be [G, n_ctx, ctx_dim]")
        Cn, L = layout.shape
        G, n_ctx = ctx.shape[0], ctx.shape[1]
        feat = torch.empty(G * Cn, self.arch.embed_dim, device=prefix.device, dtype=torch.float32)
        _lib.check(lib.mvlpt_text_fwd_grouped(self.h, _ptr(prefix), _ptr(suffix), _ptr(ctx), n_ctx, _ptr(layout), _ptr(eot),
                                              G, Cn, L, _ptr(feat), int(save_for_bwd), _stream()), self.h, "text_fwd_grouped")
        self._txt_state = (tuple(ctx.shape), layout, eot) if save_for_bwd else None
        return feat

    @_on_device
    def text_fwd_ranged(self, prefix: torch.Tensor, suffix: torch.Tensor, ctx: torch.Tensor, layout: torch.Tensor, eot: torch.Tensor,
                        class_lo, class_hi, save_for_bwd: bool = False) -> torch.Tensor:
        prefix = _req(prefix, torch.float32, "token_prefix")
        suffix = _req(suffix, torch.float32, "token_suffix")
        layout = _req(layout, torch.int32, "layout")
        eot = _req(eot, torch.int32, "eot")
        ctx = _req(ctx, torch.float32, "ctx")
        if ctx.dim() != 3:
            raise ValueError("ranged ctx must be [G, n_ctx, ctx_dim]")
        Cn, L = layout.shape
        G, n_ctx = ctx.shape[0], ctx.shape[1]
        lo, hi, S = _host_ranges(class_lo, class_hi, G, Cn)
        feat = torch.empty(S, self.arch.embed_dim, device=prefix.device, dtype=torch.float32)
        _lib.check(lib.mvlpt_text_fwd_ranged(self.h, _ptr(prefix), _ptr(suffix), _ptr(ctx), n_ctx, _ptr(layout), _ptr(eot), lo, hi,
                                             G, Cn, L, _ptr(feat), int(save_for_bwd), _stream()), self.h, "text_fwd_ranged")
        self._txt_state = (tuple(ctx.shape), layout, eot) if save_for_bwd else None
        return feat

    def load_token_embedding(self, weight: torch.Tensor) -> None:
        with torch.cuda.device(self.device):
            tg = weight.detach().float().to(self.device).contiguous()
            if tg.dim() != 2 or tg.shape[1] != self.arch.transformer_width:
                raise ValueError(f"token_embedding.weight must be [vocab, {self.arch.transformer_width}], got {tuple(tg.shape)}")
            shape = (C.c_int64 * 2)(*tg.shape)
            _lib.check(lib.mvlpt_load_frozen(self.h, b"token_embedding.weight", _ptr(tg), DT_F32, shape, 2, _stream()), self.h,
                       "load_frozen(token_embedding.weight)")
            torch.cuda.current_stream().synchronize()
        self.vocab_size = int(tg.shape[0])

    @_on_device
    def text_encode_tokens(self, ids, L: Optional[int] = None) -> torch.Tensor:
        if isinstance(ids, torch.Tensor):
# ... 606 lines not shown
```

mvlpt_amd/model.py:

```python
from __future__ import annotations

import math
import os
from collections import OrderedDict
from functools import reduce
from operator import mul
from typing import Callable, Dict, List, Optional, Sequence

import torch
import torch.nn as nn

from ._lib import TEXT_MIN_L
from .engine import Engine
from .weights import ClipArch, _randn, arch_from_state_dict

DEFAULT_TEXT_CUS = 0

SOT_TOKEN, EOT_TOKEN = 49406, 49407
X_TOKEN = 343


_DEFAULT_TOKENIZER = None


# ... 319 lines not shown
        vpt_emb_deep = None if vpt_emb.shape[0] == 1 else vpt_emb[1:, :, :]
        return coop_emb, vpt_emb[0, :, :].unsqueeze(0), vpt_emb_deep


def class_shard_bounds(n_cls: int, world: int):
    base, rem = divmod(n_cls, world)
    return [(r * base + min(r, rem), (r + 1) * base + min(r + 1, rem)) for r in range(world)]


class ClassShard:

    def __init__(self, rank: int, bounds, device, dtype=torch.float32):
        self.rank, self.bounds, self.world = rank, bounds, len(bounds)
        self.cmax = max(hi - lo for lo, hi in bounds)
        self.lo, self.hi = bounds[rank]
        self.even = all(hi - lo == self.cmax for lo, hi in bounds)
        self.device, self.dtype = device, dtype
        self._e = None
        self.slot_of_class = torch.cat([torch.arange(hi - lo) + r * self.cmax for r, (lo, hi) in enumerate(bounds)]).to(device)

    def _buffers(self, e: int):
        if self._e != e:
            z = lambda rows: torch.zeros(rows, e, device=self.device, dtype=self.dtype)
            self.gin, self.gout, self.sin, self.sout = z(self.cmax), z(self.world * self.cmax), z(self.world * self.cmax), z(self.cmax)
            self._e = e
        return self.gin, self.gout, self.sin, self.sout

    def gather(self, loc: torch.Tensor) -> torch.Tensor:
        import torch.distributed as dist
        gin, gout, _, _ = self._buffers(loc.shape[1])
        gin[:loc.shape[0]].copy_(loc)
        if dist.get_backend() == "gloo":
            h = torch.zeros(gout.shape, dtype=gout.dtype)
            h[self.rank * self.cmax:(self.rank + 1) * self.cmax] = gin.cpu()
            dist.all_reduce(h, op=dist.ReduceOp.SUM)
            gout.copy_(h)
        else:
            dist.all_gather_into_tensor(gout, gin)
        return gout if self.even else gout.index_select(0, self.slot_of_class)

    def scatter_grads(self, dtxt: torch.Tensor) -> torch.Tensor:
        import torch.distributed as dist
        _, _, sin, sout = self._buffers(dtxt.shape[1])
        if self.even:
            src = dtxt.contiguous()
        else:
            sin.index_copy_(0, self.slot_of_class, dtxt)
            src = sin
        if dist.get_backend() == "gloo":
            h = src.cpu()
            dist.all_reduce(h, op=dist.ReduceOp.SUM)
            sout.copy_(h[self.rank * self.cmax:(self.rank + 1) * self.cmax])
        else:
            dist.reduce_scatter_tensor(sout, src, op=dist.ReduceOp.SUM)
        return sout[:self.hi - self.lo]


def _text_inputs(model, pl, n_ctx):
    if not model.trim_text_to_eot:
        return pl.token_suffix, pl.layout
    L_eff = pl.max_eot + 1
    return pl.token_suffix[:, :L_eff - 1 - n_ctx], pl.layout[:, :L_eff]


class _PromptedClipFn(torch.autograd.Function):

    @staticmethod
    def forward(fctx, model: "CustomCLIP", image, task_lo, task_hi, coop_emb, vpt_emb, vpt_deep_emb, grad_on=True):
        eng = model.engine
        pl = model.prompt_learner
        need_txt = grad_on and bool(fctx.needs_input_grad[4])
        need_img = grad_on and bool(fctx.needs_input_grad[5] or fctx.needs_input_grad[6])
        ver = None
        if not pl.training and not need_txt and coop_emb is not None:
            ver = tuple((id(p), p._version) for p in model.prompt_learner.parameters())
            if model._eval_text_cache is not None and model._eval_text_cache[0] == ver:
                model._const_text_features, cached_eval = model._eval_text_cache[1], True
            else:
                cached_eval = False
        else:
            cached_eval = False
        run_text = not ((coop_emb is None or cached_eval) and model._const_text_features is not None)
        suffix, layout = _text_inputs(model, pl, pl.coop_n_ctx)
        pre = model._prefetched.pop((image.data_ptr(), tuple(image.shape), image._version), None) if vpt_emb is None else None
        if pre is not None:
            def image_fwd(*_a, **_k):
                torch.cuda.current_stream().wait_event(pre[1])
                pre[0].record_stream(torch.cuda.current_stream())
                return pre[0]
        else:
            for other in model._prefetched.values():
                torch.cuda.current_stream().wait_event(other[1])
            image_fwd = eng.image_fwd
        shard = model._class_shard if (run_text and coop_emb is not None) else None
        side = model._side_stream if (run_text and model.overlap_towers and shard is None) else None
        if shard is not None:
            lo, hi = shard.lo, shard.hi
            ctx_loc = coop_emb if coop_emb.dim() == 2 else coop_emb[lo:hi]

            def text_side():
                loc = eng.text_fwd(pl.token_prefix[lo:hi], suffix[lo:hi], ctx_loc, layout[lo:hi], pl.eot[lo:hi],
                                   save_for_bwd=need_txt)
                return shard.gather(loc)
            side_s = model._side_stream if model.overlap_towers else None
            if side_s is not None:
                main = torch.cuda.current_stream()
                side_s.wait_stream(main)
                with torch.cuda.stream(side_s):
                    txt = text_side()
                img = image_fwd(image, vpt_emb, vpt_deep_emb, save_for_bwd=need_img)
                main.wait_stream(side_s)
                txt.record_stream(main)
            else:
                img = image_fwd(image, vpt_emb, vpt_deep_emb, save_for_bwd=need_img)
                txt = text_side()
        elif side is not None:
            main = torch.cuda.current_stream()
            side.wait_stream(main)
            with torch.cuda.stream(side):
                txt = eng.text_fwd(pl.token_prefix, suffix, coop_emb, layout, pl.eot, save_for_bwd=need_txt)
            img = image_fwd(image, vpt_emb, vpt_deep_emb, save_for_bwd=need_img)
            main.wait_stream(side)
            txt.record_stream(main)
        else:
            img = image_fwd(image, vpt_emb, vpt_deep_emb, save_for_bwd=need_img)
            if run_text:
                txt = eng.text_fwd(pl.token_prefix, suffix, coop_emb, layout, pl.eot, save_for_bwd=need_txt)
        if not run_text:
            txt = model._const_text_features
        elif coop_emb is None:
            model._const_text_features = txt
        if ver is not None:
            model._eval_text_cache = (ver, txt.clone() if shard is not None else txt)
        if coop_emb is not None:
            model._const_text_features = None
        logits = eng.logits_fwd(img, txt, model.logit_scale_exp, task_lo, task_hi)
        model._fwd_generation += 1
        fctx.generation = model._fwd_generation
        fctx.model, fctx.need_img, fctx.need_txt = model, need_img, need_txt
        fctx.shard, fctx.ctx_shape = shard, (None if coop_emb is None else coop_emb.shape)
        fctx.has_deep = vpt_deep_emb is not None
        fctx.vpt_shape = None if vpt_emb is None else vpt_emb.shape
        return logits

    @staticmethod
    def backward(fctx, dlogits):
        eng = fctx.model.engine
        if fctx.generation != fctx.model._fwd_generation:
            raise RuntimeError("backward of a stale forward: the engine holds the saved activations of the most recent "
                               "CustomCLIP.forward only (call backward before the next forward)")
        dimg, dtxt = eng.logits_bwd(dlogits.contiguous(), fctx.need_img, fctx.need_txt)
        dctx = dvpt = ddeep = None
        if fctx.need_txt and fctx.shard is not None:
            lo, hi = fctx.shard.lo, fctx.shard.hi
            own = fctx.shard.scatter_grads(dtxt)
            dloc = eng.text_bwd(own)
            if len(fctx.ctx_shape) == 3:
                dctx = torch.zeros(fctx.ctx_shape, device=dloc.device, dtype=dloc.dtype)
                dctx[lo:hi] = dloc
            else:
                dctx = dloc
        elif fctx.need_txt:
            part = fctx.model._text_partition
            if part is not None and not fctx.need_img:
                main = torch.cuda.current_stream()
                part.wait_stream(main)
                with torch.cuda.stream(part):
                    dctx = eng.text_bwd(dtxt)
                dtxt.record_stream(part)
                main.wait_stream(part)
                dctx.record_stream(main)
            else:
                dctx = eng.text_bwd(dtxt)
        if fctx.need_img:
            dvpt, ddeep = eng.image_bwd(dimg)
            dvpt = dvpt.view(fctx.vpt_shape)
        return None, None, None, None, dctx, dvpt, ddeep, None


class _CrossEntropyFn(torch.autograd.Function):

    @staticmethod
    def forward(fctx, model, logits, label):
        loss, dl, nc = model.engine.cross_entropy(logits, label, need_grad=bool(fctx.needs_input_grad[1]))
        if dl is not None:
            fctx.save_for_backward(dl)
        model.last_ncorrect = nc
        return loss.squeeze(0)

    @staticmethod
    def backward(fctx, g):
        (dl,) = fctx.saved_tensors
        return None, dl * g, None


class CustomCLIP(nn.Module):

    def __init__(self, cfg, classnames, clip_model: FrozenCLIP, dm=None, pretokenized: Optional[PretokenizedPrompts] = None):
        super().__init__()
        self.prompt_learner = MultitaskVLPromptLearner(cfg, classnames, clip_model, pretokenized)
        self.tokenized_prompts = self.prompt_learner.tokenized_prompts
        self.clip_model = clip_model
        self.engine = clip_model.engine
        self.logit_scale = clip_model.logit_scale
        self.logit_scale_exp = float(clip_model.logit_scale.exp())
        self.dtype = clip_model.dtype
        self._const_text_features = None
        self.last_ncorrect = None
        self.overlap_towers = True
        self._class_shard = None
        self._eval_text_cache = None
        self.trim_text_to_eot = False
        self._prefetch_stream = None
        self._prefetched = {}
        self._fwd_generation = 0
        self._prio = os.environ.get("MVLPT_TEXT_PRIORITY", "0") != "0"
        self._side_stream = torch.cuda.Stream(device=clip_model.device, priority=-1 if self._prio else 0) if torch.cuda.is_available() else None
        self._text_partition = None
        self.text_cus = 0
        if self._side_stream is not None:
            self.set_cu_partition(int(os.environ.get("MVLPT_TEXT_CUS", DEFAULT_TEXT_CUS)))
        self.multi_task_label_pertask = cfg.DATASET.MULTITASK_LABEL_PERTASK
        if self.multi_task_label_pertask:
            start = torch.arange(dm._num_classes)
            end = torch.arange(dm._num_classes)
            s = 0
            for i, task in enumerate(dm._task_names):
                start[i] = s
                s += len(dm._labelmap[task])
                end[i] = s
            self.class_index_pertask_start, self.class_index_pertask_end = start, end

    def enable_class_sharding(self, rank: int, world: int) -> None:
        if world <= 1:
            self._class_shard = None
            return
        C = self.prompt_learner.n_cls
        if world > C:
            raise ValueError(f"class sharding needs at least one class per rank ({C} classes, {world} ranks)")
        self._class_shard = ClassShard(rank, class_shard_bounds(C, world), self.clip_model.device)

    def set_cu_partition(self, text_cus: int) -> None:
        from .engine import device_cus, partition_stream
        dev = self.clip_model.device
        pl = self.prompt_learner
        if text_cus <= 0 or pl.vpt_embeddings is not None or pl.coop_n_ctx == 0:
            if self._text_partition is not None:
                self._side_stream = torch.cuda.Stream(device=dev)
                self._prefetch_stream = None
            self._text_partition, self.text_cus = None, 0
            return
        total = device_cus(dev)
        text_cus = min(max(8, text_cus // 8 * 8), total - 8)
        torch.cuda.synchronize(dev)
        self._side_stream = self._text_partition = partition_stream(dev, 0, text_cus)
        self._prefetch_stream = partition_stream(dev, text_cus, total - text_cus)
        self.text_cus = text_cus

    def prefetch_image_features(self, image) -> bool:
        pl = self.prompt_learner
        if pl.vpt_embeddings is not None or self._side_stream is None:
            return False
        key = (image.data_ptr(), tuple(image.shape), image._version)
        if key in self._prefetched:
            return True
        main = torch.cuda.current_stream()
        if self._prefetch_stream is None:
            self._prefetch_stream = torch.cuda.Stream(device=self.clip_model.device, priority=1 if self._prio else 0)
        st = self._prefetch_stream
        ready = torch.cuda.Event()
        ready.record(main)
        st.wait_event(ready)
        with torch.cuda.stream(st):
            feat = self.engine.image_fwd(image, None, None, save_for_bwd=False)
            ev = torch.cuda.Event()
            ev.record(st)
        image.record_stream(st)
        if len(self._prefetched) >= 4:
            self._prefetched.pop(next(iter(self._prefetched)))
        self._prefetched[key] = (feat, ev, image)
        return True

    def drop_prefetch(self) -> None:
        pre, self._prefetched = self._prefetched, {}
        for entry in pre.values():
            torch.cuda.current_stream().wait_event(entry[1])

    def prompt_learner_visual_prompts(self):
        _, vpt_emb, vpt_emb_deep = self.prompt_learner.forward_mvlpt_proj(self.dtype)
        if vpt_emb is not None:
            vpt_emb = self.prompt_learner.vpt_proj(vpt_emb)
            vpt_emb_deep = None if vpt_emb_deep is None else self.prompt_learner.vpt_proj(vpt_emb_deep)
        return vpt_emb, vpt_emb_deep

    def vpt_dropout_masks(self, B):
        pl = self.prompt_learner
        p = float(pl.vpt_dropout.p)
        if pl.vpt_embeddings is None or p == 0.0 or not pl.training:
            return None
        if getattr(self, "_vpt_masks_override", None) is not None:
            return self._vpt_masks_override
        n_layers = 1 + (pl.vpt_embeddings_deep.shape[0] if (pl.vpt_deep and pl.vpt_embeddings_deep is not None) else 0)
        dev = pl.vpt_embeddings.device
        ones = torch.ones(B, pl.vpt_n_ctx, self.clip_model.arch.vision_width, device=dev)
        return torch.stack([pl.vpt_dropout(ones) for _ in range(n_layers)])

    def forward(self, image, task=None):
        coop_emb, vpt_emb, vpt_emb_deep = self.prompt_learner.forward_mvlpt_proj(self.dtype)
        if vpt_emb is not None:
            proj = self.prompt_learner.vpt_proj
            vpt_emb = proj(vpt_emb)
            if vpt_emb_deep is not None:
                vpt_emb_deep = proj(vpt_emb_deep)
            self.engine.set_vpt_dropout(self.vpt_dropout_masks(image.shape[0]))
        lo = hi = None
        if self.multi_task_label_pertask:
            t = task.cpu().long() if torch.is_tensor(task) else torch.as_tensor(task).long()
            lo = self.class_index_pertask_start[t].to(torch.int32).to(image.device)
            hi = self.class_index_pertask_end[t].to(torch.int32).to(image.device)
        return _PromptedClipFn.apply(self, image, lo, hi, coop_emb, vpt_emb, vpt_emb_deep, torch.is_grad_enabled())

    def cross_entropy(self, logits, label):
        return _CrossEntropyFn.apply(self, logits, label)
```

mvlpt_amd/mvlpt_cocoop.py:

```python
from __future__ import annotations

import math
from collections import OrderedDict
from functools import reduce
from operator import mul
from typing import List, Optional, Tuple

import torch
import torch.nn as nn

from . import _lib
from .cocoop import DEFAULT_MAX_TEXT_WORKSPACE_BYTES, MAX_SEQUENCES_PER_TOWER
from .model import FrozenCLIP, PretokenizedPrompts, _CrossEntropyFn, _text_inputs, build_prompt_layout
from .model import MultitaskVLPromptLearner as _BasePromptLearner


class MultitaskVLPromptLearner(_BasePromptLearner):

    def __init__(self, cfg, classnames, clip_model: FrozenCLIP, pretokenized: Optional[PretokenizedPrompts] = None):
        nn.Module.__init__(self)
        n_cls = len(classnames)
        T = cfg.TRAINER.MVLPT
        cocoop_n_ctx, vpt_n_ctx = T.COCOOP.N_CTX, T.VPT.N_CTX
        if cocoop_n_ctx == 0:
# ... 137 lines not shown
        need_ctx = grad_on and bool(fctx.needs_input_grad[2])
        need = need_img or need_ctx
        L = _text_inputs(model, pl, pl.cocoop_n_ctx)[1].shape[1]
        chunks = model.chunks(lo, hi, L, save_for_bwd=need)
        save = need and len(chunks) == 1
        B = ctx_shifted.shape[0]
        logits = torch.empty(B, pl.n_cls, device=img.device, dtype=torch.float32)
        for g0, g1, S in chunks:
            if S == 0:
                logits[g0:g1] = 0.0
            else:
                logits[g0:g1] = _TextSideFn._chunk_forward(model, img, ctx_shifted, lo, hi, g0, g1, save)
        if mask is not None:
            logits = logits * mask
        model.last_chunks, model.last_sequences = len(chunks), sum(c[2] for c in chunks)
        model.last_recompute = need and len(chunks) > 1
        fctx.model, fctx.lo, fctx.hi, fctx.chunks, fctx.mask = model, lo, hi, chunks, mask
        fctx.need_img, fctx.need_ctx, fctx.saved_in_engine = need_img, need_ctx, save
        fctx.generation = model._fwd_generation
        if need:
            fctx.save_for_backward(img, ctx_shifted)
        return logits

    @staticmethod
    def backward(fctx, dlogits):
        model = fctx.model
        eng = model.engine
        if fctx.saved_in_engine and fctx.generation != model._fwd_generation:
            raise RuntimeError("backward of a stale forward: the engine holds the saved activations of the most recent "
                               "CustomCLIP.forward only (call backward before the next forward)")
        img, ctx_shifted = fctx.saved_tensors
        dl = dlogits.contiguous() if fctx.mask is None else (dlogits * fctx.mask).contiguous()
        dimg = torch.zeros_like(img) if fctx.need_img else None
        dctx = torch.zeros_like(ctx_shifted) if fctx.need_ctx else None
        for g0, g1, S in fctx.chunks:
            if S == 0:
                continue
            if not fctx.saved_in_engine:
                _TextSideFn._chunk_forward(model, img, ctx_shifted, fctx.lo, fctx.hi, g0, g1, fctx.need_ctx)
            di, dtxt = eng.logits_ranged_bwd(dl[g0:g1], need_img=fctx.need_img, need_txt=fctx.need_ctx)
            if fctx.need_img:
                dimg[g0:g1] = di
            if fctx.need_ctx:
                dctx[g0:g1] = eng.text_bwd(dtxt)
        return None, dimg, dctx, None, None, None, None


class CustomCLIP(nn.Module):

    def __init__(self, cfg, classnames, clip_model: FrozenCLIP, dm=None, pretokenized: Optional[PretokenizedPrompts] = None):
        super().__init__()
        self.prompt_learner = MultitaskVLPromptLearner(cfg, classnames, clip_model, pretokenized)
        self.tokenized_prompts = self.prompt_learner.tokenized_prompts
        self.clip_model = clip_model
        self.engine = clip_model.engine
        self.logit_scale = clip_model.logit_scale
        self.logit_scale_exp = float(clip_model.logit_scale.exp())
        self.dtype = clip_model.dtype
        self.trim_text_to_eot = False
        self.ranged_text = True
        self.max_text_workspace_bytes = DEFAULT_MAX_TEXT_WORKSPACE_BYTES
        if self.engine.precision == _lib.PREC_SPLIT_GRAD:
            self.engine.set_precision("split_all")
        self.last_ncorrect = None
        self.last_chunks = self.last_sequences = 0
        self.last_recompute = False
        self._fwd_generation = 0
        self.multi_task_label_pertask = cfg.DATASET.MULTITASK_LABEL_PERTASK
        self.class_index_pertask_start = self.class_index_pertask_end = None
        if self.multi_task_label_pertask:
            start, end = torch.arange(dm._num_classes), torch.arange(dm._num_classes)
            s = 0
            for i, task in enumerate(dm._task_names):
                start[i] = s
                s += len(dm._labelmap[task])
                end[i] = s
            self.class_index_pertask_start, self.class_index_pertask_end = start, end

    def enable_class_sharding(self, rank: int, world: int) -> None:
        if world > 1:
            raise NotImplementedError("class sharding does not apply to the COCOOP.N_CTX != 0 route: every image has its own text "
                                      "features, there is no shared [n_cls, e] matrix to shard")

    def prefetch_image_features(self, image) -> bool:
        return False

    def drop_prefetch(self) -> None:
        pass

    def chunks(self, lo: List[int], hi: List[int], L: int, save_for_bwd: bool) -> List[Tuple[int, int, int]]:
        eng, budget = self.engine, self.max_text_workspace_bytes
        return chunk_bounds([b - a for a, b in zip(lo, hi)],
                            lambda S: S <= MAX_SEQUENCES_PER_TOWER and eng.text_workspace_bytes(S, L, save_for_bwd) <= budget)

    def vpt_dropout_masks(self, B):
        from .model import CustomCLIP as _Base
        return _Base.vpt_dropout_masks(self, B)

    def forward(self, image, task=None):
        pl = self.prompt_learner
        B = image.shape[0]
        self._fwd_generation += 1
        _, vpt_emb, vpt_emb_deep = pl.forward_mvlpt_proj(self.dtype)
        if vpt_emb is not None:
            proj = pl.vpt_proj
            vpt_emb = proj(vpt_emb)
            if vpt_emb_deep is not None:
                vpt_emb_deep = proj(vpt_emb_deep)
            self.engine.set_vpt_dropout(self.vpt_dropout_masks(B))
            img = _ImageTowerFn.apply(self, image, vpt_emb, vpt_emb_deep, torch.is_grad_enabled())
        else:
            img = self.engine.image_fwd(image, None, None, save_for_bwd=False)
        imf = img / img.norm(dim=-1, keepdim=True)
        ctx_shifted = pl(imf)
        lo, hi = class_ranges(task, self.class_index_pertask_start, self.class_index_pertask_end, B, pl.n_cls)
        mask = None
        if not self.ranged_text and self.multi_task_label_pertask:
            idx = torch.arange(pl.n_cls).unsqueeze(0)
            mask = ((idx >= torch.tensor(lo).unsqueeze(1)) & (idx < torch.tensor(hi).unsqueeze(1))).float().to(image.device)
            lo, hi = [0] * B, [pl.n_cls] * B
        return _TextSideFn.apply(self, img, ctx_shifted, lo, hi, mask, torch.is_grad_enabled())

    def cross_entropy(self, logits, label):
        return _CrossEntropyFn.apply(self, logits, label)
```

mvlpt_amd/trainer.py:

```python
from __future__ import annotations

import math
import os
import os.path as osp
import time
from collections import OrderedDict
from typing import Dict, Iterable, Optional

import torch

from . import distributed as dist_utils
from .config import CfgNode
from .model import CustomCLIP, FrozenCLIP
from .weights import ARCHS, make_state_dict


def build_optimizer(model: torch.nn.Module, optim_cfg, flat=None) -> torch.optim.Optimizer:
    params = [p for p in model.parameters() if p.requires_grad]
    name = optim_cfg.NAME.lower()
    if optim_cfg.get("FUSED", False):
        from .optim import FUSED
        if name not in FUSED:
            raise ValueError(f"unsupported optimizer {optim_cfg.NAME} on the fused route (sgd | adam | adamw)")
        if optim_cfg.get("AMSGRAD", False) or optim_cfg.get("STAGED_LR", False):
            raise ValueError("OPTIM.FUSED supports neither amsgrad nor staged learning rates (one param group)")
        if flat is None:
            raise ValueError("OPTIM.FUSED: build_optimizer needs flat=(FlatParameters, FlatGradients) of the model's parameters")
        if name == "sgd":
            return FUSED[name](flat[0], flat[1], lr=optim_cfg.LR, momentum=optim_cfg.MOMENTUM, weight_decay=optim_cfg.WEIGHT_DECAY,
                               dampening=optim_cfg.SGD_DAMPNING, nesterov=optim_cfg.SGD_NESTEROV)
        return FUSED[name](flat[0], flat[1], lr=optim_cfg.LR, weight_decay=optim_cfg.WEIGHT_DECAY)
    if name == "sgd":
        return torch.optim.SGD(params, lr=optim_cfg.LR, momentum=optim_cfg.MOMENTUM, weight_decay=optim_cfg.WEIGHT_DECAY,
                               dampening=optim_cfg.SGD_DAMPNING, nesterov=optim_cfg.SGD_NESTEROV)
    if name == "adam":
        return torch.optim.Adam(params, lr=optim_cfg.LR, weight_decay=optim_cfg.WEIGHT_DECAY)
    if name == "adamw":
        return torch.optim.AdamW(params, lr=optim_cfg.LR, weight_decay=optim_cfg.WEIGHT_DECAY)
    raise ValueError(f"unsupported optimizer {optim_cfg.NAME}")


def load_pretrained_weights(model: torch.nn.Module, weight_path: str) -> None:
    ck = torch.load(weight_path, map_location="cpu")
    sd = ck.get("state_dict", ck)
    own = model.state_dict()
    keep, dropped = {}, []
    for k, v in sd.items():
        k = k[7:] if k.startswith("module.") else k
        if k in ("token_prefix", "token_suffix") or k not in own or own[k].shape != v.shape:
            dropped.append(k)
            continue
        keep[k] = v
    if not keep:
        raise RuntimeError(f'The pretrained weights "{weight_path}" cannot be loaded, check the key names')
    own.update(keep)
    model.load_state_dict(own)
    if dropped:
        print(f"load_pretrained_weights: layers discarded due to unmatched keys or size: {dropped}")


class _ConstantWarmupCosine:

    def __init__(self, optim, optim_cfg):
        if optim_cfg.WARMUP_EPOCH > 0 and optim_cfg.WARMUP_TYPE not in ("constant", "linear"):
            raise ValueError(f"unsupported OPTIM.WARMUP_TYPE {optim_cfg.WARMUP_TYPE!r} (constant | linear)")
        if optim_cfg.LR_SCHEDULER != "cosine":
            raise ValueError(f"unsupported OPTIM.LR_SCHEDULER {optim_cfg.LR_SCHEDULER!r} (only cosine)")
        self.optim, self.cfg = optim, optim_cfg
        self.base_lrs = [g["lr"] for g in optim.param_groups]
        self.last_epoch = 0
        self._apply()

    def _lr(self, base):
        c = self.cfg
        W = c.WARMUP_EPOCH
        if self.last_epoch < W:
            if c.WARMUP_TYPE == "constant":
                return c.WARMUP_CONS_LR
            if self.last_epoch == 0:
                return c.WARMUP_MIN_LR
            return base * self.last_epoch / W
        return 0.5 * base * (1 + math.cos(math.pi * (self.last_epoch - W) / c.MAX_EPOCH))

    def _apply(self):
        for g, b in zip(self.optim.param_groups, self.base_lrs):
            g["lr"] = self._lr(b)

    def step(self):
        self.last_epoch += 1
        self._apply()

    def state_dict(self):
        return {"last_epoch": self.last_epoch, "base_lrs": self.base_lrs}

    def load_state_dict(self, sd):
        self.last_epoch, self.base_lrs = sd["last_epoch"], sd["base_lrs"]
        self._apply()


def build_lr_scheduler(optim, optim_cfg):
    return _ConstantWarmupCosine(optim, optim_cfg)


_PREFETCH_EARLY = os.environ.get("MVLPT_PREFETCH_EARLY", "0") != "0"


class TrainerX:

    def __init__(self, cfg: CfgNode):
        self._models, self._optims, self._scheds = OrderedDict(), OrderedDict(), OrderedDict()
        self._flat_grads, self._flat_params, self._skipped_seen = {}, {}, {}
        self.cfg = cfg
        self.rank, self.world_size, self.local_rank = dist_utils.rank_info()
        self.device = torch.device(f"cuda:{self.local_rank}") if torch.cuda.is_available() else torch.device("cpu")
        if self.device.type == "cuda":
            torch.cuda.set_device(self.device)
        dist_utils.init_process_group()
        self.start_epoch = self.epoch = 0
        self.max_epoch = cfg.OPTIM.MAX_EPOCH
        self.output_dir = cfg.OUTPUT_DIR
        self.batch_idx, self.num_batches = 0, 0
        self.next_batch, self.batch_hook = None, None
        self.check_cfg(cfg)
        self.build_data_loader()
        self.build_model()

    def register_model(self, name="model", model=None, optim=None, sched=None):
        self._models[name], self._optims[name], self._scheds[name] = model, optim, sched

    def get_model_names(self, names=None):
        return list(self._models.keys()) if names is None else list(names)

    def set_model_mode(self, mode="train", names=None):
        for n in self.get_model_names(names):
            self._models[n].train(mode == "train")

    def update_lr(self, names=None):
        for n in self.get_model_names(names):
            if self._scheds[n] is not None:
                self._scheds[n].step()

    def model_zero_grad(self, names=None):
        for n in self.get_model_names(names):
            flat = getattr(self, "_flat_grads", {}).get(n)
            if flat is not None:
                flat.zero_()
            elif self._optims[n] is not None:
                self._optims[n].zero_grad(set_to_none=False)

    def model_backward(self, loss):
        loss.backward()

    def model_update(self, names=None, loss=None):
        for n in self.get_model_names(names):
            if self._optims[n] is not None:
                if loss is not None and n in getattr(self, "_flat_params", {}):
                    self._optims[n].step(loss_dev=loss.detach())
                else:
                    self._optims[n].step()

    def model_backward_and_update(self, loss, names=None):
        self.model_zero_grad(names)
        self.model_backward(loss)
        self.sync_gradients(names)
        self.model_update(names, loss=loss)

    def sync_gradients(self, names=None):
        if self.world_size > 1:
            for n in self.get_model_names(names):
                flat = getattr(self, "_flat_grads", {}).get(n)
                if flat is not None:
                    flat.all_reduce_mean_(self.world_size)
                else:
                    dist_utils.all_reduce_gradients(self._models[n].parameters(), self.world_size)

    def flatten_gradients(self, name):
        self._flat_grads[name] = dist_utils.FlatGradients(self._models[name].parameters())
        return self._flat_grads[name]

    def build_optim(self, name, module):
        flat = None
        if self.cfg.OPTIM.get("FUSED", False):
            flat = (dist_utils.FlatParameters(module.parameters()), dist_utils.FlatGradients(module.parameters()))
        optim = build_optimizer(module, self.cfg.OPTIM, flat)
        sched = build_lr_scheduler(optim, self.cfg.OPTIM)
        self.register_model(name, module, optim, sched)
        if flat is None:
# ... 134 lines not shown
        self._task_class_idx, self._id2task = {}, {}
        if book is not None:
            self._task_names, self._labelmap = list(book._task_names), dict(book._labelmap)
            self._id2task, self._task_class_idx = dict(book._id2task), dict(book._task_class_idx)
        elif task_class_counts:
            self._task_names = [f"task{i}" for i in range(len(task_class_counts))]
            self._labelmap = {n: list(range(c)) for n, c in zip(self._task_names, task_class_counts)}
            self._id2task = dict(enumerate(self._task_names))
            lo = 0
            for n, c in zip(self._task_names, task_class_counts):
                self._task_class_idx[n] = (lo, lo + c)
                lo += c
        if elevater:
            from .metrics import get_metric
            if task_class_counts:
                names = list(metric_names or ["accuracy"] * len(task_class_counts))
                self._metric_name = dict(zip(self._task_names, names))
                self._metric = {t: get_metric(n) for t, n in self._metric_name.items()}
            else:
                self._metric_name = metric_names or "accuracy"
                self._metric = get_metric(self._metric_name)
        B, R = cfg.DATALOADER.TRAIN_X.BATCH_SIZE, cfg.INPUT.SIZE[0]
        g = torch.Generator().manual_seed(seed)
        batches = []
        for _ in range(steps_per_epoch):
            img = torch.randn(B, 3, R, R, generator=g)
            dom = torch.zeros(B, dtype=torch.long)
            if task_class_counts:
                dom = torch.randint(0, len(task_class_counts), (B,), generator=g)
                starts = torch.tensor([0] + list(torch.tensor(task_class_counts).cumsum(0)[:-1]))
                lab = starts[dom] + (torch.rand(B, generator=g) * torch.tensor(task_class_counts)[dom]).long()
            else:
                lab = torch.randint(0, num_classes, (B,), generator=g)
            if soft_labels or (elevater and (task_class_counts or self._metric_name != "accuracy")):
                lab = torch.nn.functional.one_hot(lab, num_classes).float()
            if elevater:
                batches.append((img.to(device), lab.to(device), [str(i) for i in range(B)], dom))
            else:
                batches.append({"img": img.to(device), "label": lab.to(device), "domain": dom})
        self.train_loader_x = batches
        self.train_loader_u = self.val_loader = None
        self.test_loader = batches[:1]


class MVLPT(TrainerX):

    def __init__(self, cfg, dm=None, clip_state_dict=None):
        self._dm_arg, self._sd_arg = dm, clip_state_dict
        super().__init__(cfg)

    def check_cfg(self, cfg):
        assert cfg.TRAINER.MVLPT.PREC in ["fp16", "fp32", "amp"]
        if cfg.TRAINER.MVLPT.COCOOP.N_CTX != 0:
            assert cfg.TRAINER.MVLPT.COCOOP.PREC in ["fp16", "fp32", "amp"]

    def build_data_loader(self):
        self.multi_task = self.cfg.DATASET.MULTITASK
        self.multi_task_label_pertask = self.cfg.DATASET.MULTITASK_LABEL_PERTASK
        dm = self._dm_arg
        if dm is None:
            raise ValueError("pass a data manager (e.g. SyntheticDataManager); dataset readers are out of scope")
        pipelined = self.cfg.TRAINER.MVLPT.STEP_PIPELINING and self.cfg.TRAINER.MVLPT.COCOOP.N_CTX == 0
        self.train_loader_x = LookAheadLoader(dm.train_loader_x, self) if pipelined else dm.train_loader_x
        self.train_loader_u = dm.train_loader_u
        self.val_loader, self.test_loader = dm.val_loader, dm.test_loader
        self.num_classes, self.num_source_domains, self.lab2cname = dm.num_classes, dm.num_source_domains, dm.lab2cname
        self.dm = dm

    def build_model(self):
        cfg = self.cfg
        classnames = self.dm.dataset.classnames if cfg.DATASET.COOP else list(self.dm.lab2cname.values())
        pretok = getattr(self.dm, "pretokenized", None)
        sd = self._sd_arg
        if sd is None:
            sd = make_state_dict(ARCHS[cfg.MODEL.BACKBONE.NAME], seed=cfg.SEED)
        prec = "split_all" if cfg.TRAINER.MVLPT.PREC == "fp32" else cfg.TRAINER.MVLPT.GRAD_PRECISION
        model_cls = CustomCLIP
        if cfg.TRAINER.MVLPT.COCOOP.N_CTX != 0:
            from .mvlpt_cocoop import CustomCLIP as model_cls
            if cfg.TRAINER.MVLPT.COCOOP.PREC == "fp32":
                prec = "split_all"
        clip_model = FrozenCLIP(sd, compute_dtype=cfg.TRAINER.MVLPT.COMPUTE_DTYPE, device=self.device, precision=prec)
        self.model = model_cls(cfg, classnames, clip_model, dm=self.dm, pretokenized=pretok)
        for name, param in self.model.named_parameters():
            if "prompt_learner" not in name:
                param.requires_grad_(False)
        if cfg.MODEL.INIT_WEIGHTS:
            load_pretrained_weights(self.model.prompt_learner, cfg.MODEL.INIT_WEIGHTS)
        self.model.to(self.device)
        if self.world_size > 1:
            dist_utils.broadcast_parameters(self.model.prompt_learner)
        self.optim, self.sched = self.build_optim("prompt_learner", self.model.prompt_learner)
        self.scaler = None

    def forward_backward(self, batch):
        next_batch = self.next_batch if self.cfg.TRAINER.MVLPT.STEP_PIPELINING else None
        ahead = getattr(self, "_parsed_ahead", None)
        if ahead is not None and ahead[0] is batch:
            image, label, tasks_ = ahead[1]
        else:
            image, label, tasks_ = self.parse_batch_train(batch)
        self._parsed_ahead = None
        if len(label.shape) > 1 and label.shape[-1] > 1:
            label = label.float()
            label = label / label.sum(dim=-1, keepdim=True)
        early = next_batch is not None and _PREFETCH_EARLY
        if early:
            parsed = self.parse_batch_train(next_batch)
            self._parsed_ahead = (next_batch, parsed)
            self.model.prefetch_image_features(parsed[0])
        output = self.model(image, task=tasks_)
        loss = self.model.cross_entropy(output, label)
        if next_batch is not None and not early:
            parsed = self.parse_batch_train(next_batch)
            self._parsed_ahead = (next_batch, parsed)
            self.model.prefetch_image_features(parsed[0])
        self.model_backward_and_update(loss)
        loss_summary = {"loss": loss.detach(), "acc": self.model.last_ncorrect[0] * (100.0 / output.shape[0])}
        if tasks_ is not None:
            loss_summary["num_tasks"] = len(set(tasks_.tolist()))
        if (self.batch_idx + 1) == self.num_batches:
            self.update_lr()
        return loss_summary

    def end_of_epoch_loop(self):
        super().end_of_epoch_loop()
        self._parsed_ahead = None
        if getattr(self, "model", None) is not None:
            self.model.drop_prefetch()

    def after_epoch(self):
        super().after_epoch()
        self.model.engine.trim()

    def parse_batch_train(self, batch):
        if self.cfg.DATASET.COOP:
            inp_key, lab_key, task_key = "img", "label", "domain"
        else:
            inp_key, lab_key, task_key = 0, 1, 3
        tasks = batch[task_key] if self.multi_task else None
        return batch[inp_key].to(self.device), batch[lab_key].to(self.device), tasks

    parse_batch_test = parse_batch_train

    @torch.no_grad()
    def model_inference(self, input, task=None):
        return self.model(input, task=task)

    @torch.no_grad()
    def test(self, split=None):
        self.set_model_mode("eval")
        split = split or self.cfg.TEST.SPLIT
        loader = self.val_loader if (split == "val" and self.val_loader is not None) else self.test_loader
        if loader is None:
            raise RuntimeError(f"test(split={split!r}): the data manager has no val/test loader; set TEST.NO_TEST True for "
                               "runs without evaluation data")
        coop = self.cfg.DATASET.COOP
        correct = torch.zeros((), device=self.device)
        total = 0
        per_task = {}
        y_pred, y_true, y_task = [], [], []
        for batch in loader:
            input, label, tasks_ = self.parse_batch_test(batch)
            output = self.model_inference(input, task=tasks_)
            if not coop:
                y_pred.append(output.float())
                y_true.append(label)
                if tasks_ is not None:
                    y_task.append(torch.as_tensor(tasks_).cpu())
                continue
            if label.dim() > 1:
                label = label.argmax(dim=1)
            correct += (output.argmax(dim=1) == label).sum()
            total += label.shape[0]
            if tasks_ is not None and self._task_ranges() is not None:
                ranges = self._task_ranges()
                for t_id in set(tasks_.tolist()):
                    sel = (tasks_ == t_id).to(output.device)
                    lo, hi = ranges[t_id]
                    hit = (output[sel][:, lo:hi].argmax(dim=1) + lo == label[sel]).sum()
                    acc = per_task.setdefault(t_id, [torch.zeros((), device=self.device), 0])
                    acc[0] += hit
                    acc[1] += int(sel.sum())
        results_overall = {}
        if coop:
            results = {"accuracy": 100.0 * float(correct) / max(total, 1)}
            results_overall = {self.dm._task_names[t]: 100.0 * float(c) / max(n, 1) for t, (c, n) in per_task.items()}
        else:
            import numpy as np
            pred = torch.cat(y_pred).cpu().numpy()
            true = torch.cat(y_true).cpu().numpy()
            if y_task:
                task_ids = torch.cat(y_task).numpy()
                for t_id in sorted(set(task_ids.tolist())):
                    task = self.dm._id2task[t_id]
                    lo, hi = self.dm._task_class_idx[task]
                    yt, yp = true[task_ids == t_id][:, lo:hi], pred[task_ids == t_id][:, lo:hi]
                    if self.dm._metric_name[task] == "accuracy":
# ... 36 lines not shown
```

Measured before the change: 19300 images/sec.

## Split next-batch image prefetch into capped early blocks and a resumed tail

Adds begin/resume entry points to the image forward so the next batch's prefetch can run its first blocks (default 6) early, on a side stream whose CU count is capped (default 192) and so sized for fewer workgroups. This lets them overlap the current step's text forward. The remaining blocks are resumed after the loss, before backward. The aim is to fill idle compute while the current step's smaller text-tower and head kernels run, without starving them. The risk is contention and reduced parallelism in the capped kernels, plus extra state-machine complexity around pending forwards.

Result: faster. 19570 images/sec, median of 6 (+1.4%).

```diff
diff --git a/include/mvlpt_hip.h b/include/mvlpt_hip.h
--- a/include/mvlpt_hip.h
+++ b/include/mvlpt_hip.h
@@ -34,6 +34,7 @@
 int mvlpt_stream_create_cus(int cu_first, int cu_count, mvlpt_stream_t* stream);
 int mvlpt_stream_destroy(mvlpt_stream_t stream);
 int mvlpt_stream_cus(mvlpt_stream_t stream);
+int mvlpt_stream_set_cu_cap(mvlpt_stream_t stream, int n);
 
 int mvlpt_load_frozen(void* handle, const char* name, const void* dev_ptr, int dtype, const int64_t* shape, int ndim,
                       mvlpt_stream_t stream);
@@ -41,6 +42,10 @@
 
 int mvlpt_image_fwd(void* handle, const void* image, int image_dtype, const float* vpt, const float* vpt_deep, int n_vpt,
                     int n_deep, int B, float* feat_out, int save_for_bwd, mvlpt_stream_t stream);
+int mvlpt_image_fwd_begin(void* handle, const void* image, int image_dtype, const float* vpt, const float* vpt_deep, int n_vpt,
+                          int n_deep, int B, int save_for_bwd, int stop_block, mvlpt_stream_t stream);
+int mvlpt_image_fwd_resume(void* handle, float* feat_out, mvlpt_stream_t stream);
+int mvlpt_image_fwd_abandon(void* handle);
 int mvlpt_image_bwd(void* handle, const float* dfeat, float* dvpt, float* dvpt_deep, mvlpt_stream_t stream);
 
 int mvlpt_text_fwd(void* handle, const float* prefix, const float* suffix, const float* ctx, int ctx_per_class, int n_ctx,
diff --git a/mvlpt_amd/_lib.py b/mvlpt_amd/_lib.py
--- a/mvlpt_amd/_lib.py
+++ b/mvlpt_amd/_lib.py
@@ -13,6 +13,7 @@
 EPI_STORE16, EPI_GELU, EPI_RESID32, EPI_GELUBWD, EPI_STORE32, EPI_GELU_SPLIT, EPI_GELUBWD_SPLIT, EPI_STORE_SPLIT = 0, 1, 2, 3, 4, 5, 6, 7
 GEMM_BT_128x128_R2, GEMM_BT_128x128_R4, GEMM_BT_256x128_R3, GEMM_BT_256x256_R2, GEMM_PHASED, GEMM_PC, GEMM_PCP = 1, 2, 3, 4, 5, 6, 7
 PREC_FAST, PREC_SPLIT_GRAD, PREC_SPLIT_ALL = 0, 1, 2
+ERR_ARG, ERR_HIP, ERR_STATE, ERR_UNSUPPORTED = -1, -2, -3, -4
 TEXT_MIN_L = 3
 
 
@@ -62,9 +63,13 @@
     "mvlpt_stream_create_cus": (_i, [_i, _i, C.POINTER(_vp)]),
     "mvlpt_stream_destroy": (_i, [_vp]),
     "mvlpt_stream_cus": (_i, [_vp]),
+    "mvlpt_stream_set_cu_cap": (_i, [_vp, _i]),
     "mvlpt_load_frozen": (_i, [_vp, C.c_char_p, _vp, _i, C.POINTER(C.c_int64), _i, _vp]),
     "mvlpt_frozen_ready": (_i, [_vp]),
     "mvlpt_image_fwd": (_i, [_vp, _vp, _i, _vp, _vp, _i, _i, _i, _vp, _i, _vp]),
+    "mvlpt_image_fwd_begin": (_i, [_vp, _vp, _i, _vp, _vp, _i, _i, _i, _i, _i, _vp]),
+    "mvlpt_image_fwd_resume": (_i, [_vp, _vp, _vp]),
+    "mvlpt_image_fwd_abandon": (_i, [_vp]),
     "mvlpt_image_bwd": (_i, [_vp, _vp, _vp, _vp, _vp]),
     "mvlpt_text_fwd": (_i, [_vp, _vp, _vp, _vp, _i, _i, _vp, _vp, _i, _i, _vp, _i, _vp]),
     "mvlpt_text_bwd": (_i, [_vp, _vp, _vp, _vp]),
diff --git a/mvlpt_amd/config.py b/mvlpt_amd/config.py
--- a/mvlpt_amd/config.py
+++ b/mvlpt_amd/config.py
@@ -63,6 +63,8 @@
         COMPUTE_DTYPE="fp16",
         GRAD_PRECISION="split_grad",
         STEP_PIPELINING=True,
+        PREFETCH_SPLIT=(6, 192),
+        PREFETCH_SPLIT_TOWERS=("ViT-B/16",),
     )
     cfg.TRAINER.COCOOP = CN(N_CTX=16, CTX_INIT="", PREC="fp16")
     cfg.TRAINER.ZSCLIP = CN(TEMPLATES=["a photo of a {}."])
diff --git a/mvlpt_amd/csrc/attention.hip b/mvlpt_amd/csrc/attention.hip
--- a/mvlpt_amd/csrc/attention.hip
+++ b/mvlpt_amd/csrc/attention.hip
@@ -653,7 +653,7 @@
   if (use_stream(a.L)) return launch_attn_fwd_stream(dtype, a, s);
   if (!a.causal && a.q_rows <= 0 && (a.L + 15) / 16 == PNT && (dtype == DT_F16 || dtype == DT_BF16)) {
     const int total = a.N * a.H, cus = stream_cus(s);
-    if (total >= 2 * cus) {
+    if (total >= 2 * stream_cus_nocap(s)) {
       static bool set = false;
       if (!set) {
         hipFuncSetAttribute((const void*)attn_fwdp_kernel<f16>, hipFuncAttributeMaxDynamicSharedMemorySize, PLDS);
diff --git a/mvlpt_amd/csrc/attention32.hip b/mvlpt_amd/csrc/attention32.hip
--- a/mvlpt_amd/csrc/attention32.hip
+++ b/mvlpt_amd/csrc/attention32.hip
@@ -1166,7 +1166,7 @@
   }
   if (attn32_resident(a.L, a.causal)) {
     const int total = a.N * a.H, cus = stream_cus(s);
-    if (a.q_rows <= 0 && total >= 2 * cus) {
+    if (a.q_rows <= 0 && total >= 2 * stream_cus_nocap(s)) {
       static bool setp = false;
       if (!setp) { set_lds(attn32p_fwd_kernel<T>, RLDS_P); setp = true; }
       hipLaunchKernelGGL((attn32p_fwd_kernel<T>), dim3(cus), dim3(RNW * 64), RLDS_P, s, a, total);
diff --git a/mvlpt_amd/csrc/engine.hip b/mvlpt_amd/csrc/engine.hip
--- a/mvlpt_amd/csrc/engine.hip
+++ b/mvlpt_amd/csrc/engine.hip
@@ -20,6 +20,7 @@
 struct StreamPart { hipStream_t s; int cus; };
 std::mutex g_part_mu;
 std::vector<StreamPart> g_parts;
+std::vector<StreamPart> g_caps;
 int device_cus() {
   static int cus = 0;
   if (!cus) {
@@ -31,13 +32,18 @@
 }
 }
 namespace mvlpt {
-int stream_cus(hipStream_t s) {
+static int stream_cus_impl(hipStream_t s, bool capped) {
+  int cus = 0, cap = 0;
   if (s) {
     std::lock_guard<std::mutex> lk(g_part_mu);
-    for (const StreamPart& p : g_parts) if (p.s == s) return p.cus;
-  }
-  return device_cus();
-}
+    for (const StreamPart& p : g_parts) if (p.s == s) { cus = p.cus; break; }
+    if (capped) for (const StreamPart& p : g_caps) if (p.s == s) { cap = p.cus; break; }
+  }
+  if (!cus) cus = device_cus();
+  return cap > 0 && cap < cus ? cap : cus;
+}
+int stream_cus(hipStream_t s) { return stream_cus_impl(s, true); }
+int stream_cus_nocap(hipStream_t s) { return stream_cus_impl(s, false); }
 }
 
 namespace {
@@ -142,6 +148,7 @@
   TowerState vs, ts;
   int vB = 0, v_nvpt = 0, v_ndeep = 0; float* cls32 = nullptr; float* dcls32 = nullptr;
   float* xc32 = nullptr; void *ac16 = nullptr, *hc16 = nullptr, *gc16 = nullptr;
+  struct ImgPending { bool active = false, packed = false, ln1_ready = false, save = false; int next = 0; const float* vpt_deep = nullptr; } ip;
   bool v_cls_last = false; float *xcm32 = nullptr, *xco32 = nullptr, *dxc32 = nullptr, *dhc32 = nullptr;
   void *uc16 = nullptr, *duc16 = nullptr, *dxc16 = nullptr, *dOc16 = nullptr;
   int tC = 0, tL = 0, t_nctx = 0, t_per_class = 0; int32_t* eot_rows = nullptr; int32_t* ctx_pos = nullptr;
@@ -643,6 +650,7 @@
   {
     std::lock_guard<std::mutex> lk(g_part_mu);
     for (size_t i = 0; i < g_parts.size(); ++i) if (g_parts[i].s == s) { g_parts.erase(g_parts.begin() + i); break; }
+    for (size_t i = 0; i < g_caps.size(); ++i) if (g_caps[i].s == s) { g_caps.erase(g_caps.begin() + i); break; }
   }
   hipError_t e = hipStreamDestroy(s);
   if (e != hipSuccess) return hipfail(nullptr, e, "hipStreamDestroy");
@@ -650,6 +658,21 @@
 }
 
 int mvlpt_stream_cus(mvlpt_stream_t stream) { return stream_cus((hipStream_t)stream); }
+
+int mvlpt_stream_set_cu_cap(mvlpt_stream_t stream, int n) {
+  hipStream_t s = (hipStream_t)stream;
+  if (!s) return fail(nullptr, MVLPT_ERR_ARG, "stream_set_cu_cap: the NULL stream cannot be capped");
+  if (n > 0 && n < 8) return fail(nullptr, MVLPT_ERR_ARG, "stream_set_cu_cap: a cap is at least 8 compute units (one per XCD)");
+  const int cap = n > 0 ? n / 8 * 8 : 0;
+  std::lock_guard<std::mutex> lk(g_part_mu);
+  for (size_t i = 0; i < g_caps.size(); ++i)
+    if (g_caps[i].s == s) {
+      if (cap > 0) g_caps[i].cus = cap; else g_caps.erase(g_caps.begin() + i);
+      return 0;
+    }
+  if (cap > 0) g_caps.push_back(StreamPart{s, cap});
+  return 0;
+}
 
 int mvlpt_set_resid_packed(void* h, int on) {
   Engine* E = (Engine*)h;
@@ -797,16 +820,50 @@
   return 0;
 }
 
-int mvlpt_image_fwd(void* h, const void* image, int image_dtype, const float* vpt, const float* vpt_deep, int n_vpt, int n_deep,
-                    int B, float* feat_out, int save_for_bwd, mvlpt_stream_t stream) {
-  Engine* E = (Engine*)h;
-  if (!E || !image || !feat_out || B <= 0) return fail(E, MVLPT_ERR_ARG, "image_fwd: null/invalid argument");
+static int image_blocks(Engine* E, int from, int to, bool packed, bool* ln1_ready, const float* vpt_deep, hipStream_t s) {
+  TowerState& st = E->vs;
+  const int B = E->vB, n_vpt = E->v_nvpt, n_deep = E->v_ndeep, dv = E->arch.vision_width, Lv = st.L;
+  const float* const masks = E->v_mask;
+  auto vmask = [&](int l) -> const float* { return masks ? masks + (size_t)l * B * n_vpt * dv : nullptr; };
+  auto next_foldable = [&](int l) -> const LNp* {
+    const int n = l + 1;
+    if (!st.fold || n >= E->vis.layers) return nullptr;
+    if (n_deep > 0) return nullptr;
+    return &E->vis.blocks[n].ln1;
+  };
+  for (int l = from; l < to; ++l) {
+    if (l > 0 && n_deep > 0) {
+      if (l <= n_deep) {
+        ProfScope ps(E, s, PC_GLUE, 0, (double)B * n_vpt * dv * 4.0);
+        HIPCHK(E, launch_overwrite_rows(vpt_deep + (size_t)(l - 1) * n_vpt * dv, n_vpt, st.x[2 * l], B, Lv, dv, s, vmask(l)));
+      } else {
+        st.skip[l] = 1;
+        if (st.saved) {
+          HIPCHK(E, hipMemcpyAsync(st.x[2 * l + 2], st.x[2 * l], (size_t)B * Lv * dv * 4, hipMemcpyDeviceToDevice, s));
+        }
+        continue;
+      }
+    }
+    if (l == E->vis.layers - 1) return 1;
+    if (packed) { if (int rc = block_fwd_packed(E, E->vis, st, l, s)) return rc; continue; }
+    bool produced = false;
+    if (int rc = block_fwd(E, E->vis, st, l, s, *ln1_ready, next_foldable(l), &produced)) return rc;
+    *ln1_ready = produced;
+  }
+  return 0;
+}
+
+int mvlpt_image_fwd_begin(void* h, const void* image, int image_dtype, const float* vpt, const float* vpt_deep, int n_vpt, int n_deep,
+                          int B, int save_for_bwd, int stop_block, mvlpt_stream_t stream) {
+  Engine* E = (Engine*)h;
+  if (!E || !image || B <= 0) return fail(E, MVLPT_ERR_ARG, "image_fwd: null/invalid argument");
+  if (E->ip.active) return fail(E, MVLPT_ERR_STATE, "image_fwd_begin: a forward is pending (call image_fwd_resume or image_fwd_abandon first)");
   if (int rc = mvlpt_frozen_ready(h)) return rc;
   if ((n_vpt > 0) != (vpt != nullptr)) return fail(E, MVLPT_ERR_ARG, "image_fwd: vpt pointer and n_vpt disagree");
   if ((n_deep > 0) != (vpt_deep != nullptr) || (n_deep > 0 && n_vpt <= 0)) return fail(E, MVLPT_ERR_ARG, "image_fwd: deep prompts need vpt");
   hipStream_t s = (hipStream_t)stream;
   const MvlptArch& A = E->arch;
-  const int G = A.image_resolution / A.patch_size, G2 = G * G, dv = A.vision_width, e = A.embed_dim;
+  const int G = A.image_resolution / A.patch_size, G2 = G * G, dv = A.vision_width;
   const int Lv = 1 + n_vpt + G2;
   if (Lv > attn_max_len()) return fail(E, MVLPT_ERR_UNSUPPORTED, "image_fwd: sequence length > 256 not supported yet");
   const bool save = save_for_bwd != 0;
@@ -842,7 +899,7 @@
   if (masks && (n_vpt <= 0 || mask_layers < 1 + n_deep || mask_B != B || mask_n != n_vpt))
     return fail(E, MVLPT_ERR_ARG, "image_fwd: the prompt dropout masks do not match this forward (layers >= 1 + n_deep, batch, n_vpt)");
   E->v_mask = masks;
-  auto vmask = [&](int l) -> const float* { return masks ? masks + (size_t)l * B * n_vpt * dv : nullptr; };
+  const float* const vmask0 = masks;
   { ProfScope ps(E, s, PC_GLUE, 0, (double)npatch * E->Kp * 6.0);
     HIPCHK(E, launch_patchify(E->dt, image, image_dtype, patches, B, A.image_resolution, A.patch_size, E->Kp, s)); }
   if (E->dbg_ck_on) { E->dbg_ck_n = 0; if (E->dbg_ck) (void)hipMemsetAsync(E->dbg_ck, 0, DBG_CK_MAX * sizeof(unsigned long long), s); }
@@ -861,35 +918,39 @@
     dbg_ck(E, xhi, (size_t)B * Lv * dv * 3, s); dbg_ck(E, st.part[0], (size_t)B * Lv * ntp_d * 8, s);
   } else {
     ProfScope ps(E, s, PC_GLUE, 0, (double)B * Lv * dv * 8.0);
-    HIPCHK(E, launch_assemble_tokens(pe, E->cls_emb, E->vpos, E->ln_pre.g, E->ln_pre.b, vpt, n_vpt, st.x[0], B, G2, dv, s, vmask(0)));
-  }
-  bool cls_only_last = false;
+    HIPCHK(E, launch_assemble_tokens(pe, E->cls_emb, E->vpos, E->ln_pre.g, E->ln_pre.b, vpt, n_vpt, st.x[0], B, G2, dv, s, vmask0));
+  }
+  const int stop = std::min(std::max(stop_block, 0), E->vis.layers - 1);
   bool ln1_ready = packed;
-  auto next_foldable = [&](int l) -> const LNp* {
-    const int n = l + 1;
-    if (!st.fold || n >= E->vis.layers) return nullptr;
-    if (n_deep > 0) return nullptr;
-    return &E->vis.blocks[n].ln1;
-  };
-  for (int l = 0; l < E->vis.layers; ++l) {
-    if (l > 0 && n_deep > 0) {
-      if (l <= n_deep) {
-        ProfScope ps(E, s, PC_GLUE, 0, (double)B * n_vpt * dv * 4.0);
-        HIPCHK(E, launch_overwrite_rows(vpt_deep + (size_t)(l - 1) * n_vpt * dv, n_vpt, st.x[2 * l], B, Lv, dv, s, vmask(l)));
-      } else {
-        st.skip[l] = 1;
-        if (st.saved) {
-          HIPCHK(E, hipMemcpyAsync(st.x[2 * l + 2], st.x[2 * l], (size_t)B * Lv * dv * 4, hipMemcpyDeviceToDevice, s));
-        }
-        continue;
-      }
-    }
-    if (l == E->vis.layers - 1) { cls_only_last = true; break; }
-    if (packed) { if (int rc = block_fwd_packed(E, E->vis, st, l, s)) return rc; continue; }
-    bool produced = false;
-    if (int rc = block_fwd(E, E->vis, st, l, s, ln1_ready, next_foldable(l), &produced)) return rc;
-    ln1_ready = produced;
-  }
+  if (int rc = image_blocks(E, 0, stop, packed, &ln1_ready, vpt_deep, s)) return rc;
+  E->ip.active = true; E->ip.packed = packed; E->ip.ln1_ready = ln1_ready; E->ip.save = save; E->ip.next = stop; E->ip.vpt_deep = vpt_deep;
+  return 0;
+}
+
+int mvlpt_image_fwd_abandon(void* h) {
+  Engine* E = (Engine*)h;
+  if (!E) return MVLPT_ERR_ARG;
+  if (E->ip.active) { E->ip.active = false; E->vs.valid = false; }
+  return 0;
+}
+
+int mvlpt_image_fwd_resume(void* h, float* feat_out, mvlpt_stream_t stream) {
+  Engine* E = (Engine*)h;
+  if (!E || !feat_out) return fail(E, MVLPT_ERR_ARG, "image_fwd_resume: null argument");
+  if (!E->ip.active) return fail(E, MVLPT_ERR_STATE, "image_fwd_resume: call image_fwd_begin first");
+  E->ip.active = false;
+  hipStream_t s = (hipStream_t)stream;
+  TowerState& st = E->vs;
+  const MvlptArch& A = E->arch;
+  const int B = E->vB, dv = A.vision_width, e = A.embed_dim, Lv = st.L;
+  const bool save = E->ip.save, packed = E->ip.packed;
+  const size_t X = st.exact ? 2 : 1;
+  void* const xhi = st.x[0];
+  uint8_t* const xlo = (uint8_t*)st.x[0] + (size_t)B * Lv * dv * 2;
+  bool ln1_ready = E->ip.ln1_ready;
+  const int rest = image_blocks(E, E->ip.next, E->vis.layers, packed, &ln1_ready, E->ip.vpt_deep, s);
+  if (rest < 0) { st.valid = false; return rest; }
+  const bool cls_only_last = rest == 1;
   if (cls_only_last) {
     const int l = E->vis.layers - 1;
     const Block& Bk = E->vis.blocks[l];
@@ -931,10 +992,19 @@
   return 0;
 }
 
+int mvlpt_image_fwd(void* h, const void* image, int image_dtype, const float* vpt, const float* vpt_deep, int n_vpt, int n_deep,
+                    int B, float* feat_out, int save_for_bwd, mvlpt_stream_t stream) {
+  Engine* E = (Engine*)h;
+  if (!E || !image || !feat_out || B <= 0) return fail(E, MVLPT_ERR_ARG, "image_fwd: null/invalid argument");
+  if (int rc = mvlpt_image_fwd_begin(h, image, image_dtype, vpt, vpt_deep, n_vpt, n_deep, B, save_for_bwd, E->vis.layers, stream)) return rc;
+  return mvlpt_image_fwd_resume(h, feat_out, stream);
+}
+
 int mvlpt_image_bwd(void* h, const float* dfeat, float* dvpt, float* dvpt_deep, mvlpt_stream_t stream) {
   Engine* E = (Engine*)h;
   if (!E || !dfeat) return fail(E, MVLPT_ERR_ARG, "image_bwd: null argument");
   TowerState& st = E->vs;
+  if (E->ip.active) return fail(E, MVLPT_ERR_STATE, "image_bwd: a forward is pending between image_fwd_begin and image_fwd_resume");
   if (!st.valid || !st.saved) return fail(E, MVLPT_ERR_STATE, "image_bwd: call image_fwd(save_for_bwd=1) first");
   if ((E->v_nvpt > 0 && !dvpt) || (E->v_ndeep > 0 && !dvpt_deep)) return fail(E, MVLPT_ERR_ARG, "image_bwd: missing gradient output");
   hipStream_t s = (hipStream_t)stream;
diff --git a/mvlpt_amd/csrc/kernels.h b/mvlpt_amd/csrc/kernels.h
--- a/mvlpt_amd/csrc/kernels.h
+++ b/mvlpt_amd/csrc/kernels.h
@@ -7,6 +7,7 @@
 namespace mvlpt {
 
 int stream_cus(hipStream_t s);
+int stream_cus_nocap(hipStream_t s);
 
 enum GemmEpi {
   EPI_STORE16 = 0,
diff --git a/mvlpt_amd/engine.py b/mvlpt_amd/engine.py
--- a/mvlpt_amd/engine.py
+++ b/mvlpt_amd/engine.py
@@ -50,6 +50,14 @@
 def device_cus(device: torch.device) -> int:
     with torch.cuda.device(device):
         return int(lib.mvlpt_stream_cus(None))
+
+
+def set_stream_cu_cap(stream: "torch.cuda.Stream", n: int) -> None:
+    _lib.check(lib.mvlpt_stream_set_cu_cap(C.c_void_p(stream.cuda_stream), int(n)), None, "stream_set_cu_cap")
+
+
+def stream_cus(stream: Optional["torch.cuda.Stream"] = None) -> int:
+    return int(lib.mvlpt_stream_cus(C.c_void_p(stream.cuda_stream) if stream is not None else _stream()))
 
 
 def _host_ranges(class_lo, class_hi, G: int, n_cls: int):
@@ -96,6 +104,7 @@
         self.precision = _lib.PREC_SPLIT_GRAD
         self._keep: List[torch.Tensor] = []
         self._img_state = None
+        self._img_pending = None
         self._txt_state = None
         self._head_state = None
 
@@ -162,9 +171,7 @@
                 torch.cuda.current_stream().synchronize()
             _lib.check(lib.mvlpt_frozen_ready(self.h), self.h, "frozen_ready")
 
-    @_on_device
-    def image_fwd(self, image: torch.Tensor, vpt: Optional[torch.Tensor] = None, vpt_deep: Optional[torch.Tensor] = None,
-                  save_for_bwd: bool = False) -> torch.Tensor:
+    def _image_args(self, image, vpt, vpt_deep):
         if image.dtype not in _TORCH2DT:
             image = image.float()
         image = image.contiguous()
@@ -181,12 +188,49 @@
         if vpt_deep is not None:
             vpt_deep = _req(vpt_deep, torch.float32, "vpt_deep")
             n_deep = vpt_deep.shape[0]
+        return image, vpt, vpt_deep, n_vpt, n_deep, B, m
+
+    @_on_device
+    def image_fwd(self, image: torch.Tensor, vpt: Optional[torch.Tensor] = None, vpt_deep: Optional[torch.Tensor] = None,
+                  save_for_bwd: bool = False) -> torch.Tensor:
+        image, vpt, vpt_deep, n_vpt, n_deep, B, m = self._image_args(image, vpt, vpt_deep)
         feat = torch.empty(B, self.arch.embed_dim, device=image.device, dtype=torch.float32)
         _lib.check(lib.mvlpt_image_fwd(self.h, _ptr(image), _TORCH2DT[image.dtype], _ptr(vpt), _ptr(vpt_deep), n_vpt, n_deep, B,
                                        _ptr(feat), int(save_for_bwd), _stream()), self.h, "image_fwd")
         self._img_state = (n_vpt, n_deep, B) if save_for_bwd else None
         self._vpt_masks_saved, self._vpt_masks = (m if save_for_bwd else None), None
         return feat
+
+    @_on_device
+    def image_fwd_begin(self, image: torch.Tensor, vpt: Optional[torch.Tensor] = None, vpt_deep: Optional[torch.Tensor] = None,
+                        save_for_bwd: bool = False, stop_block: Optional[int] = None) -> None:
+        image, vpt, vpt_deep, n_vpt, n_deep, B, m = self._image_args(image, vpt, vpt_deep)
+        stop = self.arch.vision_layers if stop_block is None else int(stop_block)
+        _lib.check(lib.mvlpt_image_fwd_begin(self.h, _ptr(image), _TORCH2DT[image.dtype], _ptr(vpt), _ptr(vpt_deep), n_vpt, n_deep, B,
+                                             int(save_for_bwd), stop, _stream()), self.h, "image_fwd_begin")
+        self._img_state = None
+        self._img_pending = (image, vpt, vpt_deep, m, (n_vpt, n_deep, B) if save_for_bwd else None)
+        self._vpt_masks = None
+
+    @_on_device
+    def image_fwd_resume(self) -> torch.Tensor:
+        pend = self._img_pending
+        if pend is None:
+            raise RuntimeError("image_fwd_resume without image_fwd_begin")
+        image, _vpt, _deep, m, state = pend
+        feat = torch.empty(image.shape[0], self.arch.embed_dim, device=image.device, dtype=torch.float32)
+        self._img_pending = None
+        _lib.check(lib.mvlpt_image_fwd_resume(self.h, _ptr(feat), _stream()), self.h, "image_fwd_resume")
+        self._img_state = state
+        self._vpt_masks_saved = m if state is not None else None
+        return feat
+
+    def image_fwd_pending(self) -> bool:
+        return self._img_pending is not None
+
+    def image_fwd_abandon(self) -> None:
+        _lib.check(lib.mvlpt_image_fwd_abandon(self.h), self.h, "image_fwd_abandon")
+        self._img_pending = None
 
     @_on_device
     def image_bwd(self, dfeat: torch.Tensor) -> Tuple[Optional[torch.Tensor], Optional[torch.Tensor]]:
diff --git a/mvlpt_amd/model.py b/mvlpt_amd/model.py
--- a/mvlpt_amd/model.py
+++ b/mvlpt_amd/model.py
@@ -425,7 +425,10 @@
             cached_eval = False
         run_text = not ((coop_emb is None or cached_eval) and model._const_text_features is not None)
         suffix, layout = _text_inputs(model, pl, pl.coop_n_ctx)
-        pre = model._prefetched.pop((image.data_ptr(), tuple(image.shape), image._version), None) if vpt_emb is None else None
+        key = (image.data_ptr(), tuple(image.shape), image._version)
+        if model._pending is not None and (vpt_emb is not None or key not in model._prefetched):
+            model._resume_pending()
+        pre = model._prefetched.pop(key, None) if vpt_emb is None else None
         if pre is not None:
             def image_fwd(*_a, **_k):
                 torch.cuda.current_stream().wait_event(pre[1])
@@ -556,6 +559,8 @@
         self.trim_text_to_eot = False
         self._prefetch_stream = None
         self._prefetched = {}
+        self._pending = None
+        self.prefetch_split = (0, 0)
         self._fwd_generation = 0
         self._prio = os.environ.get("MVLPT_TEXT_PRIORITY", "0") != "0"
         self._side_stream = torch.cuda.Stream(device=clip_model.device, priority=-1 if self._prio else 0) if torch.cuda.is_available() else None
@@ -600,7 +605,27 @@
         self._prefetch_stream = partition_stream(dev, text_cus, total - text_cus)
         self.text_cus = text_cus
 
-    def prefetch_image_features(self, image) -> bool:
+    def split_active(self) -> bool:
+        layers = getattr(getattr(self.engine, "arch", None), "vision_layers", 0)
+        return (0 < self.prefetch_split[0] <= layers - 1 and self.overlap_towers and self._side_stream is not None
+                and self._class_shard is None and self.text_cus == 0 and self.prompt_learner.vpt_embeddings is None)
+
+    def has_prefetched(self, image) -> bool:
+        return (image.data_ptr(), tuple(image.shape), image._version) in self._prefetched
+
+    def _resume_pending(self) -> None:
+        key, image, _ = self._pending
+        self._pending = None
+        st = self._prefetch_stream
+        with torch.cuda.stream(st):
+            feat = self.engine.image_fwd_resume()
+            ev = torch.cuda.Event()
+            ev.record(st)
+        if len(self._prefetched) >= 4:
+            self._prefetched.pop(next(iter(self._prefetched)))
+        self._prefetched[key] = (feat, ev, image)
+
+    def prefetch_image_features(self, image, stop_block=None, cu_cap=None) -> bool:
         pl = self.prompt_learner
         if pl.vpt_embeddings is not None or self._side_stream is None:
             return False
@@ -614,6 +639,24 @@
         ready = torch.cuda.Event()
         ready.record(main)
         st.wait_event(ready)
+        if self._pending is not None:
+            mine = self._pending[0] == key
+            self._resume_pending()
+            if mine:
+                return True
+        if stop_block and self.split_active():
+            from .engine import set_stream_cu_cap
+            with torch.cuda.stream(st):
+                set_stream_cu_cap(st, int(cu_cap or 0))
+                try:
+                    self.engine.image_fwd_begin(image, None, None, save_for_bwd=False, stop_block=int(stop_block))
+                finally:
+                    set_stream_cu_cap(st, 0)
+                ev = torch.cuda.Event()
+                ev.record(st)
+            image.record_stream(st)
+            self._pending = (key, image, ev)
+            return True
         with torch.cuda.stream(st):
             feat = self.engine.image_fwd(image, None, None, save_for_bwd=False)
             ev = torch.cuda.Event()
@@ -625,6 +668,10 @@
         return True
 
     def drop_prefetch(self) -> None:
+        if self._pending is not None:
+            self.engine.image_fwd_abandon()
+            torch.cuda.current_stream().wait_event(self._pending[2])
+            self._pending = None
         pre, self._prefetched = self._prefetched, {}
         for entry in pre.values():
             torch.cuda.current_stream().wait_event(entry[1])
diff --git a/mvlpt_amd/mvlpt_cocoop.py b/mvlpt_amd/mvlpt_cocoop.py
--- a/mvlpt_amd/mvlpt_cocoop.py
+++ b/mvlpt_amd/mvlpt_cocoop.py
@@ -243,7 +243,10 @@
             raise NotImplementedError("class sharding does not apply to the COCOOP.N_CTX != 0 route: every image has its own text "
                                       "features, there is no shared [n_cls, e] matrix to shard")
 
-    def prefetch_image_features(self, image) -> bool:
+    def prefetch_image_features(self, image, stop_block=None, cu_cap=None) -> bool:
+        return False
+
+    def split_active(self) -> bool:
         return False
 
     def drop_prefetch(self) -> None:
diff --git a/mvlpt_amd/trainer.py b/mvlpt_amd/trainer.py
--- a/mvlpt_amd/trainer.py
+++ b/mvlpt_amd/trainer.py
@@ -2,6 +2,7 @@
 
 import math
 import os
+import re
 import os.path as osp
 import time
 from collections import OrderedDict
@@ -103,6 +104,21 @@
 
 
 _PREFETCH_EARLY = os.environ.get("MVLPT_PREFETCH_EARLY", "0") != "0"
+
+
+def prefetch_split(cfg) -> tuple:
+    env = os.environ.get("MVLPT_PREFETCH_SPLIT", "")
+    if env:
+        m = re.fullmatch(r"\s*(\d+)\s*:\s*(\d+)\s*", env)
+        if m is None:
+            raise ValueError(f"MVLPT_PREFETCH_SPLIT={env!r}: expected k:c, two non-negative integers (stop_block:cu_cap, e.g. 6:192; "
+                             "0:0 keeps the image tower in one piece)")
+        return int(m.group(1)), int(m.group(2))
+    towers = tuple(cfg.TRAINER.MVLPT.PREFETCH_SPLIT_TOWERS)
+    if towers and cfg.MODEL.BACKBONE.NAME not in towers:
+        return 0, 0
+    k, c = cfg.TRAINER.MVLPT.PREFETCH_SPLIT
+    return max(int(k), 0), max(int(c), 0)
 
 
 class TrainerX:
@@ -403,6 +419,7 @@
                 prec = "split_all"
         clip_model = FrozenCLIP(sd, compute_dtype=cfg.TRAINER.MVLPT.COMPUTE_DTYPE, device=self.device, precision=prec)
         self.model = model_cls(cfg, classnames, clip_model, dm=self.dm, pretokenized=pretok)
+        self.model.prefetch_split = prefetch_split(cfg)
         for name, param in self.model.named_parameters():
             if "prompt_learner" not in name:
                 param.requires_grad_(False)
@@ -426,15 +443,22 @@
             label = label.float()
             label = label / label.sum(dim=-1, keepdim=True)
         early = next_batch is not None and _PREFETCH_EARLY
-        if early:
+        stop_block, cu_cap = getattr(self.model, "prefetch_split", (0, 0))
+        split = (next_batch is not None and not early and stop_block > 0 and self.model.split_active()
+                 and self.model.has_prefetched(image))
+        if early or split:
             parsed = self.parse_batch_train(next_batch)
             self._parsed_ahead = (next_batch, parsed)
-            self.model.prefetch_image_features(parsed[0])
+            if split:
+                self.model.prefetch_image_features(parsed[0], stop_block=stop_block, cu_cap=cu_cap)
+            else:
+                self.model.prefetch_image_features(parsed[0])
         output = self.model(image, task=tasks_)
         loss = self.model.cross_entropy(output, label)
         if next_batch is not None and not early:
-            parsed = self.parse_batch_train(next_batch)
-            self._parsed_ahead = (next_batch, parsed)
+            if not split:
+                parsed = self.parse_batch_train(next_batch)
+                self._parsed_ahead = (next_batch, parsed)
             self.model.prefetch_image_features(parsed[0])
         self.model_backward_and_update(loss)
         loss_summary = {"loss": loss.detach(), "acc": self.model.last_ncorrect[0] * (100.0 / output.shape[0])}
```
